# robertknight/ocrs-models

Hardware: AMD Instinct MI355X
Metric: detection train-step images/sec (higher is better)
Workload: dtype bf16

## Files before the change

include/ocrs_hip.h:

```cpp
#ifndef OCRS_HIP_H
#define OCRS_HIP_H

#ifdef __cplusplus
extern "C" {
#endif

#ifndef __HIP_PLATFORM_AMD__
typedef struct ihipStream_t* hipStream_t;
#endif

int ocrs_pack_frags(const float* src, int mode, int K, int M, int K2, long s1, long s2, long sm, void* out, int dtype, hipStream_t st);
long ocrs_pack_frags_bytes(int K, int M, int dtype);
int ocrs_pack_frags_multi(const long long* table, int n, long max_frag_threads, int dtype, hipStream_t st);

int ocrs_dwpw_fwd(const void* xa, const void* xb, int Ca, int Cb, const float* tra, const float* trb, const float* wdw, const void* wpk,
                  void* z, double* gstat, const float* gamma, void* pooled, int Cout, int N, int H, int W, int dtype, hipStream_t st);
long ocrs_dwpw_fwd_fin_supported(int Cin, int Cout, int dtype);
int ocrs_dwpw_fwd_fin(const void* xa, const void* xb, int Ca, int Cb, const float* tra, const float* trb, const float* wdw, const void* wpk, void* z,
                      double* gstat, unsigned* counter, long count, const float* bn_w, const float* bn_b, float eps, float momentum, float* tr, float* saved,
                      float* run_mean, float* run_var, long long* nbt, float lo, int Cout, int N, int H, int W, int dtype, hipStream_t st);
long ocrs_dwpw_fwd_pool_supported(int Cin, int Cout);
long ocrs_rs32_fwd_supported(int Ca, int Cb, int Cout, int dtype);
int ocrs_rs32_fwd(const float* xa, const float* xb, int Ca, int Cb, const float* tra, const float* trb, const float* wdw, const float* wpw, float* z,
                  double* gstat, const float* gamma, float* pooled, unsigned* counter, long count, const float* bn_w, const float* bn_b, float eps,
                  float momentum, float* tr, float* saved, float* run_mean, float* run_var, long long* nbt, float lo, int Cout, int N, int H, int W,
                  hipStream_t st);
long ocrs_rs32_bwd_supported(int Ca, int Cb, int Cout, int pooled, int dtype);
long ocrs_rs32_bwd_ws_floats(int Ca, int Cb, int Cout, int N, int H, int W);
int ocrs_rs32_bwd(const float* xa, const float* xb, int Ca, int Cb, const float* tra, const float* trb, const float* wdw, const float* wpw, const float* g1,
                  const float* g2, const float* z, const float* bn, const double* gsum, const float* gamma, const float* saved, float* dgamma, float* dbeta,
                  float* gxa, float* gxb, float* dwpw, float* dwdw, float* ws, const float* saved_a, double* gsum_a, const float* saved_b, double* gsum_b,
                  int pooled, int Cout, int N, int H, int W, hipStream_t st);
long ocrs_rs32_bwd_head_supported(int Ca, int Cb, int Cout, int dtype);
int ocrs_rs32_bwd_head(const float* xa, int Ca, const float* tra, const float* wdw, const float* wpw, const float* gl, const float* whead, const float* z,
                       const float* bn, const double* gsum, const float* gamma, const float* saved, float* dgamma, float* dbeta, float* gxa, float* dwpw,
                       float* dwdw, float* ws, const float* saved_a, double* gsum_a, int Cout, int N, int H, int W, hipStream_t st);
long ocrs_mm_fwd_supported(int Ca, int Cb, int Cout, int dtype);
long ocrs_mm_fwd_nparts(int Ca, int Cb, int Cout, int N, int H, int W);
int ocrs_mm_fwd(const void* xa, const void* xb, int Ca, int Cb, const float* tra, const float* trb, const float* wdw, const float* wpw, void* z,
                float* ws, const float* gamma, void* pooled, int Cout, int N, int H, int W, int dtype, hipStream_t st);
int ocrs_mm_fwd_fin(const void* xa, const void* xb, int Ca, int Cb, const float* tra, const float* trb, const float* wdw, const float* wpw, void* z, float* ws,
                    const float* gamma, void* pooled, unsigned* counter, long count, const float* bn_w, const float* bn_b, float eps, float momentum, float* tr,
                    float* saved, float* run_mean, float* run_var, long long* nbt, float lo, int Cout, int N, int H, int W, int dtype, hipStream_t st);
int ocrs_mm_fwd_fin_xu(const void* xu, const float* wexp, const float* tra, const float* wdw, const float* wpw, void* z, float* ws, unsigned* counter, long count,
                       const float* bn_w, const float* bn_b, float eps, float momentum, float* tr, float* saved, float* run_mean, float* run_var, long long* nbt,
                       float lo, int Cout, int N, int H, int W, int dtype, hipStream_t st);
int ocrs_bn_finalize_parts(const float* parts, int nparts, long count, int C, const float* gamma, const float* beta, float eps, float momentum,
                           float* tr, float* saved, float* run_mean, float* run_var, long long* nbt, float lo, hipStream_t st);
int ocrs_dwpw_c1_fwd(const float* img, const float* wdw, const float* wpw, void* z, double* gstat, int N, int H, int W, int dtype,
                     hipStream_t st);
long ocrs_dwpw_c1_u_supported(int N, int H, int W, int dtype);
int ocrs_dwpw_c1_fwd_u(const float* img, const float* wdw, const float* wpw, void* z, void* uplane, double* gstat, int N, int H, int W, int dtype,
                       hipStream_t st);
int ocrs_bn_finalize(const double* gstat, long count, int C, const float* gamma, const float* beta, float eps, float momentum, float* tr,
                     float* saved, float* run_mean, float* run_var, long long* nbt, float lo, hipStream_t st);
int ocrs_maxpool_fwd(const void* z, const float* tr, void* out, int C, int N, int H, int W, int raw, int dtype, hipStream_t st);
int ocrs_convt_fwd(const void* x, const float* tr, const void* wpk, const float* bias, void* out, int Cup, int Cout, int N, int h, int w,
                   int H, int W, int dtype, hipStream_t st);
long ocrs_rs32_convt_fwd_supported(int Cup, int Cout, int dtype);
int ocrs_rs32_convt_fwd(const float* x, const float* tr, const float* wt, const float* bias, float* out, int Cup, int Cout, int N, int h, int w, int H, int W,
                        hipStream_t st);
long ocrs_rs32_convt_dgrad_supported(int Cup, int Cout, int dtype);
int ocrs_rs32_convt_dgrad(const float* g, const float* wt, float* dx, const float* x, const float* tr, const float* saved, double* gsum, int Cup, int Cout, int N,
                          int h, int w, int H, int W, hipStream_t st);
int ocrs_head_fwd(const void* z, const float* tr, const float* w, const float* b, float* pred, long P, int dtype, hipStream_t st);

int ocrs_bn_bwd_reduce(const void* g1, const void* g2, int pooled, const void* z, const float* bn, const float* saved, double* gsum, int C,
                       int N, int H, int W, int dtype, hipStream_t st);
int ocrs_bn_bwd_finalize(const double* gsum, long count, int C, const float* gamma, const float* saved, float* coef, float* dgamma,
                         float* dbeta, hipStream_t st);
long ocrs_pw_bwd_ws_floats(int Cin, int Cout, int N, int H, int W);
int ocrs_pw_bwd(const void* xa, const void* xb, int Ca, int Cb, const float* tra, const float* trb, const float* wdw, const void* g1,
                const void* g2, int pooled, const void* z, const float* bn, const float* coef, const void* wpk_d, void* du, float* dwpw,
                float* ws, int Cout, int N, int H, int W, int dtype, hipStream_t st);
int ocrs_pw_bwd_fin(const void* xa, const void* xb, int Ca, int Cb, const float* tra, const float* trb, const float* wdw, const void* g1, const void* g2,
                    int pooled, const void* z, const float* bn, float* coef, const double* gsum, const float* gamma, const float* saved, float* dgamma,
                    float* dbeta, const void* wpk_d, void* du, float* dwpw, float* ws, int Cout, int N, int H, int W, int dtype, hipStream_t st);
long ocrs_pw_bwd_kernel(int Ca, int Cb, int Cout, int dtype);
long ocrs_dw_bwd_ws_floats(int C, int N, int H, int W);
int ocrs_dw_bwd(const void* xa, const void* xb, int Ca, int Cb, const float* tra, const float* trb, const float* wdw, const void* du,
                void* gxa, void* gxb, float* dwdw, float* ws, const float* saved_a, double* gsum_a, const float* saved_b, double* gsum_b,
                int N, int H, int W, int dtype, hipStream_t st);
long ocrs_mm_bwd_supported(int Ca, int Cb, int Cout, int dtype);
long ocrs_mm_bwd_ws_floats(int Ca, int Cb, int Cout, int N, int H, int W);
int ocrs_mm_bwd(const void* xa, const void* xb, int Ca, int Cb, const float* tra, const float* trb, const float* wdw, const float* wpw,
                const void* g1, const void* g2, int pooled, const void* z, const float* bn, const float* coef, void* gxa, void* gxb, float* dwpw,
                float* dwdw, float* ws, const float* saved_a, double* gsum_a, const float* saved_b, double* gsum_b, int Cout, int N, int H,
                int W, int dtype, hipStream_t st);
int ocrs_mm_bwd_fin(const void* xa, const void* xb, int Ca, int Cb, const float* tra, const float* trb, const float* wdw, const float* wpw, const void* g1,
                    const void* g2, int pooled, const void* z, const float* bn, const double* gsum, const float* gamma, const float* saved, float* dgamma,
                    float* dbeta, void* gxa, void* gxb, float* dwpw, float* dwdw, float* ws, const float* saved_a, double* gsum_a, const float* saved_b,
                    double* gsum_b, int Cout, int N, int H, int W, int dtype, hipStream_t st);
long ocrs_mm_bwd_head_supported(int Ca, int Cb, int Cout, int N, int H, int W, int dtype);
int ocrs_mm_bwd_fin_head(const void* xa, int Ca, const float* tra, const float* wdw, const float* wpw, const float* gl, const float* whead, const void* z,
                         const float* bn, const double* gsum, const float* gamma, const float* saved, float* dgamma, float* dbeta, void* gxa, float* dwpw,
                         float* dwdw, float* ws, const float* saved_a, double* gsum_a, int Cout, int N, int H, int W, int dtype, hipStream_t st);
int ocrs_mm_bwd_fin_xu(const void* xu, const float* wexp, const float* tra, const float* wdw, const float* wpw, const void* g1, const void* g2, const void* z,
                       const float* bn, const double* gsum, const float* gamma, const float* saved, float* dgamma, float* dbeta, void* gxa, float* dwpw,
                       float* dwdw, float* ws, const float* saved_a, double* gsum_a, int Cout, int N, int H, int W, int dtype, hipStream_t st);
int ocrs_dwpw_c1_bwd(const float* img, const float* wdw, const float* wpw, const void* g1, const void* g2, int pooled, const void* z,
                     const float* bn, const float* coef, double* acc64, int N, int H, int W, int dtype, hipStream_t st);
long ocrs_convt_bwd_ws_floats(int Cup, int Cout, int N, int h, int w, int dtype);
int ocrs_convt_bwd(const void* x, const float* tr, const void* g, const void* wpk_d, void* dx, float* dW, float* dbias, double* dbias64, float* ws,
                   const float* saved, double* gsum, int Cup, int Cout, int N, int h, int w, int H, int W, int dtype, hipStream_t st);
long ocrs_convt_bwd_stats_supported(int Cup, int Cout, int dtype);
long ocrs_convt_bwd_splittable(int Cup, int Cout, int dtype);
int ocrs_convt_bwd_parts(const void* x, const float* tr, const void* g, const void* wpk_d, void* dx, float* dW, float* dbias, double* dbias64, float* ws,
                         const float* saved, double* gsum, int Cup, int Cout, int N, int h, int w, int H, int W, int parts, int dtype, hipStream_t st);
int ocrs_dwpw_c1_fwd_us(const float* img, const float* wdw, const float* wpw, void* z, void* uplane, double* gstat, double* fsum, int N, int H, int W, int dtype,
                        hipStream_t st);
int ocrs_mm_bwd_fin_xu_c1(const void* xu, const float* wexp, const float* tra, const float* wdw, const float* wpw, const void* g1, const void* g2, const void* z,
                          const float* bn, const double* gsum, const float* gamma, const float* saved, float* dgamma, float* dbeta, float* dwpw, float* dwdw,
                          float* ws, const float* saved_a, double* gsum_a, const float* img, double* c1acc, int Cout, int N, int H, int W, int dtype,
                          hipStream_t st);
int ocrs_c1_bwd_fin(const double* c1acc, const double* fsum, const float* coef, const float* wexp, double* acc64, hipStream_t st);
int ocrs_bwd_defer_begin(double* scratch, long ndoubles);
int ocrs_bwd_defer_flush(hipStream_t st);
int ocrs_head_bwd(const void* z, const float* tr, const float* w, const float* pred, const float* gpred, void* gy, double* acc64,
                  const float* saved, double* gsum, long P, int dtype, hipStream_t st);
int ocrs_head_bwd_gl(const void* z, const float* tr, const float* w, const float* pred, const float* gpred, float* gl, double* acc64,
                     const float* saved, double* gsum, long P, int dtype, hipStream_t st);
int ocrs_head_bwd_loss(const void* z, const float* tr, const float* w, const float* pred, const float* target, const float* lpx, const unsigned char* cls,
                       const void* state, const float* gout, float* gl, double* acc64, const float* saved, double* gsum, long P, int dtype,
                       hipStream_t st);

long ocrs_loss_state_bytes(void);
long ocrs_loss_hist_bytes(void);
int ocrs_balanced_bce_fwd(const float* pred, const float* target, float* lpx, unsigned char* cls, void* state, void* hist, float* loss_out,
                          long P, hipStream_t st);
int ocrs_balanced_bce_bwd(const float* pred, const float* target, const float* lpx, const unsigned char* cls, const void* state,
                          const float* gout, float* gpred, long P, hipStream_t st);
int ocrs_fold64_multi(const int* table, int nrows, float* dst, const double* src, hipStream_t st);

int ocrs_conv_igemm(const void* x, int ldx, const void* wpk, void* out, int ldo, const float* bias, int relu, double* gstat, int Cin, int M, int N,
                    int Hi, int Wi, int Ho, int Wo, int KH, int KW, int padh, int padw, int dtype, hipStream_t st);
long ocrs_conv_igemm_kernel(int ldx, int ldo, int Cin, int M, int Hi, int Wi, int Ho, int Wo, int KH, int KW, int padh, int padw, int dtype);
long ocrs_wgrad_gemm_x3_ws_floats(int CA, int CB, long P);
int ocrs_wgrad_gemm_x3(const float* A, int ldA, int CA, const float* B, int ldB, int CB, float* dW, float* ws, long P, hipStream_t st);
int ocrs_gemm_x3(const float* X, int ldx, int K, const float* Wm, int ldw, int km, const float* bias, float* out, int ldo, int M, long P, int Kw,
                 hipStream_t st);
long ocrs_gemm_x3p_supported(int ldx, int K, int ldo, int M, long P);
int ocrs_gemm_x3p(const float* X, int ldx, int K, const void* wpk, const float* bias, float* out, int ldo, int M, long P, hipStream_t st);
int ocrs_gemm_x3p_tiles(const float* X, int ldx, int K, const void* wpk, const float* bias, float* out, int ldo, int M, long P, int ntw, hipStream_t st);
long ocrs_wgrad_gather_ws_floats(int CA, int CB, int ntaps, long P, int dtype);
int ocrs_wgrad_gather(const void* A, int ldA, int CA, const float* trA, const void* B, int ldB, int CB, float* dW, float* ws, int N, int hA,
                      int wA, int HB, int WB, int stride, int padh, int padw, int KH, int KW, int dtype, hipStream_t st);
long ocrs_conv3x3_wgrad_ws_floats(int Cout, int Cin, int N, int H, int W);
int ocrs_conv3x3_wgrad(const void* dz, int Cout, const void* x, int Cin, float* dW, float* ws, int N, int H, int W, int dtype, hipStream_t st);
int ocrs_conv0_fwd(const float* img, const float* w, const float* bias, void* out, int N, int H, int W, int dtype, hipStream_t st);
int ocrs_conv0_bwd(const float* img, const float* w, const float* bias, const void* g, float* dW, float* db, int N, int H, int W, int dtype,
                   hipStream_t st);
int ocrs_act_pool_fwd(const void* z, const float* tr, void* out, int C, int N, int H, int W, int PH, int PW, int dtype, hipStream_t st);
int ocrs_rec_bn_reduce(const void* g, const void* z, const float* bn, const float* saved, double* gsum, int C, int N, int H, int W, int PH, int PW,
                       int dtype, hipStream_t st);
int ocrs_dz_apply(const void* g, const void* z, const float* bn, const float* coef, void* dz, int C, int N, int H, int W, int PH, int PW, int dtype,
                  float* dsum , hipStream_t st);
int ocrs_avgpool_fwd(const void* z, const float* tr, float* seq, int C, int N, int H, int W, int dtype, hipStream_t st);
int ocrs_avgpool_bn_reduce(const float* gseq, const void* z, const float* saved, double* gsum, int C, int N, int H, int W, int dtype, hipStream_t st);
int ocrs_avgpool_dz(const float* gseq, const void* z, const float* coef, void* dz, int C, int N, int H, int W, int dtype, hipStream_t st);
int ocrs_col_sum(const void* a, int ld, int C, float* out, long rows, int dtype, hipStream_t st);
int ocrs_gru_layer_fwd(const float* gi, const float* whh_pk, const float* bhh, float* out, float* saved, int T, int N, hipStream_t st);
int ocrs_gru_layer_bwd(const float* dout, const float* saved, const float* out, const float* whhT_pk, float* dgi, float* dgh, float* dhz, int T,
                       int N, hipStream_t st);
long ocrs_gru_seq_supported(int N);
long ocrs_gru_seq_sync_words(int N);
long ocrs_gru_seq_ws_floats(int N);
int ocrs_gru_seq_fwd(const float* gi, const float* whh, const float* bhh, float* out, float* saved, int T, int N, unsigned* sync, unsigned* err, float* xws,
                     int exact, hipStream_t st);
int ocrs_gru_seq_bwd(const float* dout, const float* saved, const float* out, const float* whh, float* dgi, float* dgh, int T, int N, unsigned* sync,
                     unsigned* err, float* xws, int exact, float* dbih, float* dbhh, hipStream_t st);
int ocrs_gru_seq_status(const unsigned* err, hipStream_t st);
int ocrs_log_softmax_fwd(const void* logits, float* out, long rows, int C, int ld, int dtype, hipStream_t st);
int ocrs_log_softmax_bwd(const float* lp, const float* g, void* dlogits, long rows, int C, int ld, int dtype, hipStream_t st);
int ocrs_ctc_fwd(const float* lp, const int* targets, const long long* in_len, const long long* tg_len, float* alpha, float* nll, float* loss,
                 int T, int N, int C, int Lpad, int Smax, hipStream_t st);
int ocrs_ctc_bwd(const float* lp, const int* targets, const long long* in_len, const long long* tg_len, const float* alpha, const float* nll,
                 const float* gout, float* grad, int T, int N, int C, int Lpad, int Smax, hipStream_t st);
int ocrs_ctc_fwd_ab(const float* lp, const int* targets, const long long* in_len, const long long* tg_len, float* alpha, float* beta, float* nll,
                    float* loss, int T, int N, int C, int Lpad, int Smax, hipStream_t st);
int ocrs_ctc_grad_ab(const float* lp, const int* targets, const long long* in_len, const long long* tg_len, const float* alpha, const float* beta,
                     const float* nll, const float* gout, float* grad, int T, int N, int C, int Lpad, int Smax, hipStream_t st);
int ocrs_ctc_fwd_h16(const float* lp, const int* targets, const long long* in_len, const long long* tg_len, void* alpha16, float* rowmax, float* nll,
                     float* loss, int T, int N, int C, int Lpad, int Smax, hipStream_t st);
int ocrs_ctc_bwd_h16(const float* lp, const int* targets, const long long* in_len, const long long* tg_len, const void* alpha16, const float* rowmax,
                     const float* nll, const float* gout, float* grad, int T, int N, int C, int Lpad, int Smax, hipStream_t st);
int ocrs_ctc_greedy_decode(const float* lp, const long long* in_len, int* amax, int* labels, int* lens, int T, int N, int C, hipStream_t st);
long ocrs_edit_distance_ws_bytes(int N, int pa);
int ocrs_edit_distance(const int* a, const long long* a_len, int pa, const int* b, const long long* b_len, int pb, const int* codes, int ncodes,
                       void* ws, int* dist, int N, hipStream_t st);
long ocrs_ctc_cer_ws_bytes(int T, int N, int Lpitch);
int ocrs_ctc_cer_update(const float* lp, const long long* in_len, const int* targets, const long long* tgt_len, const int* codes, void* ws,
                        long long* state, int* dist, int T, int N, int C, int Lpitch, hipStream_t st);

int ocrs_transform_image_u8(const void* img_u8, void* out, long n, int dtype, hipStream_t st);
int ocrs_collate_pad(const void* packed, const long long* offs, const int* widths, void* out, int B, int H, int Wpad, int kind, int dtype,
                     hipStream_t st);
int ocrs_resize_aa(const float* in, float* ws, float* out, int planes, int h, int w, int oh, int ow, hipStream_t st);
long ocrs_resize_aa_ws_floats(int planes, int h, int ow);

long ocrs_augment_det_ws_floats(int B);
int ocrs_augment_det(const void* img_u8, const void* mask, const long long* offs, const int* params, float* ws, void* img_out, float* mask_out,
                     int B, int max_h, int max_w, int OH, int OW, int mask_kind, int dtype, hipStream_t st);
long ocrs_augment_lines_ws_floats(int B, long inter_floats, long hpass_floats);
int ocrs_augment_lines(const void* crops, const void* masks, const long long* offs, const int* params, float* ws, long inter_floats, void* out, int B,
                       int max_ih, int max_iw, int OH, int Wpad, int kind, int clamp, int dtype, hipStream_t st);

long ocrs_cc_quads_capacity(int H, int W);
long ocrs_cc_quads_ws_bytes(int B, int H, int W);
int ocrs_cc_quads(const void* mask, int kind, float threshold, int B, int H, int W, int* ncomp, float* quads, int* labels, void* ws,
                  hipStream_t st);
long ocrs_box_match_ws_bytes(int B, long cap_t, int nbkt);
int ocrs_box_match_metrics(const float* pred_quads, const int* n_pred, long cap_p, const float* target_quads, const int* n_target, long cap_t, int B,
                           int nbkt, double* out, void* ws, hipStream_t st);
long ocrs_mask_metrics_ws_bytes(int B, int H, int W);
int ocrs_mask_metrics(const void* pred, int pred_kind, const void* target, int target_kind, float threshold, int B, int H, int W, double* out, void* ws,
                      hipStream_t st);

int ocrs_binarize_resize_nearest(const float* prob, unsigned char* out, int B, int h, int w, int H, int W, float threshold, hipStream_t st);
int ocrs_expand_quads(const float* quads, float* out, const int* counts, int B, long cap, float dist, hipStream_t st);
int ocrs_crop_plan(const float* quads, const int* count, long cap, int output_height, int* plan, long long* totals, hipStream_t st);
int ocrs_rectify_crops(const unsigned char* page, int H, int W, const float* quads, const int* plan, const long long* totals, long max_tiles, float* packed,
                       long packed_floats, hipStream_t st);
long ocrs_resize_aa_packed_ws_floats(long hpass_floats);
int ocrs_resize_aa_packed(const float* packed, const int* plan, const int* count, long cap, const long long* chunks, int nchunks, int max_batch, float* ws,
                          long ws_floats, float* out, long out_floats, int output_height, hipStream_t st);

long ocrs_text_lines_ws_bytes(long cap);
int ocrs_line_links(const float* quads, const int* count, long cap, float max_gap, float min_cos, int* next_word, void* ws, long ws_bytes, hipStream_t st);
int ocrs_line_rank(const int* count, long cap, const int* next_word, void* ws, long ws_bytes, hipStream_t st);
int ocrs_line_order(const int* count, long cap, int* n_lines, int* line_of_word, int* word_order, int* line_offsets, void* ws, long ws_bytes, hipStream_t st);
int ocrs_line_quads(const float* quads, const int* count, long cap, const int* n_lines, const int* line_offsets, const int* word_order, float* line_quads,
                    void* ws, long ws_bytes, hipStream_t st);

int ocrs_binarize_resize_pages(const float* prob, const int* page_sizes, unsigned char* out, int B, int h, int w, int Hmax, int Wmax, float threshold,
                               hipStream_t st);
int ocrs_gather_page_quads(const float* quads, const int* counts, int B, long cap, float* out, int* page_of_word, int* word_offs, long out_cap, hipStream_t st);
long ocrs_text_lines_pages_ws_bytes(long cap, int B);
int ocrs_line_links_pages(const float* quads, const int* word_offs, int B, long cap, float max_gap, float min_cos, int* next_word, void* ws, long ws_bytes,
                          hipStream_t st);
int ocrs_line_rank_pages(const int* word_offs, int B, long cap, const int* next_word, void* ws, long ws_bytes, hipStream_t st);
int ocrs_line_order_pages(const int* word_offs, int B, long cap, int* n_lines, int* line_of_word, int* word_order, int* line_offsets, int* line_page_offs,
                          int* page_of_line, void* ws, long ws_bytes, hipStream_t st);
int ocrs_line_quads_pages(const float* quads, const int* word_offs, int B, long cap, const int* n_lines, const int* line_offsets, const int* word_order,
                          float* line_quads, void* ws, long ws_bytes, hipStream_t st);
int ocrs_rectify_crops_pages(const unsigned char* pages, long pages_bytes, const long long* page_offs, const int* page_sizes, int B, const float* quads,
                             const int* page_of_quad, const int* plan, const long long* totals, long max_tiles, float* packed, long packed_floats,
                             hipStream_t st);

long ocrs_tile_batch_ws_floats(int T, int max_th, int ow);
int ocrs_tile_batch(const unsigned char* pages, long pages_bytes, const long long* page_offs, const int* page_sizes, int B, const int* tiles, int T, int max_th,
                    float* ws, long ws_floats, float* out, int oh, int ow, hipStream_t st);
#define OCRS_TILES_AXIS_MAX 64
int ocrs_binarize_resize_tiles(const float* prob, int T, int h, int w, const int* tiles, const int* tile_offs, const int* page_sizes, const int* grids,
                               const int* row_cuts, const int* col_cuts, int max_axis, unsigned char* out, int B, int Hmax, int Wmax, float threshold,
                               hipStream_t st);

long ocrs_reading_order_ws_bytes(long cap, int B);
int ocrs_reading_relation(const float* line_quads, const int* n_lines, const int* line_page_offs , int B, long cap, unsigned* before,
                          void* ws, long ws_bytes, hipStream_t st);
int ocrs_reading_peel(const int* n_lines, const int* line_page_offs, int B, long cap, const unsigned* before, int* line_order, void* ws, long ws_bytes,
                      hipStream_t st);
int ocrs_reading_blocks(const int* n_lines, const int* line_page_offs, int B, long cap, float block_gap, const int* line_order, int* new_block, void* ws,
                        long ws_bytes, hipStream_t st);

int ocrs_ctc_decode_spans(const float* lp, const long long* in_len, int* amax, float* amax_lp, int T, int N, int C, long row0, int ld, int* labels, int* t0, int* t1,
                          float* peak, int* lens, hipStream_t st);
int ocrs_char_boxes(const float* quads, const int* plan, long cap, long rows, int ld, const int* lens, const int* t0, const int* t1, float* s0, float* s1,
                    float* char_quads, hipStream_t st);
int ocrs_word_chars(const float* words, long wcap, const float* line_quads, const int* n_lines, long cap, const int* line_offsets, const int* word_order,
                    const int* plan, long rows, int ld, const int* labels, const int* lens, const float* s0, const float* s1, int space, int* word_chars,
                    hipStream_t st);

int ocrs_line_spines(const float* words, long wcap, const int* n_lines, long cap, const int* line_offsets, const int* word_order, float* spine, float* line_dims,
                     hipStream_t st);
int ocrs_crop_plan_dims(const float* line_dims, const int* count, long cap, int output_height, int* plan, long long* totals, hipStream_t st);
int ocrs_rectify_chain(const unsigned char* page, int H, int W, const float* spine, const float* line_dims, const int* line_offsets, long wcap, const int* plan,
                       const long long* totals, long max_tiles, float* packed, long packed_floats, hipStream_t st);
int ocrs_rectify_chain_pages(const unsigned char* pages, long pages_bytes, const long long* page_offs, const int* page_sizes, int B, const float* spine,
                             const float* line_dims, const int* line_offsets, long wcap, const int* page_of_line, const int* plan, const long long* totals,
                             long max_tiles, float* packed, long packed_floats, hipStream_t st);
int ocrs_char_boxes_chain(const float* spine, const float* line_dims, const int* line_offsets, long wcap, const int* plan, long cap, long rows, int ld,
                          const int* lens, const int* t0, const int* t1, float* s0, float* s1, float* char_quads, hipStream_t st);
int ocrs_word_chars_chain(const float* spine, long wcap, const int* n_lines, long cap, const int* line_offsets, const int* word_order, const int* plan, long rows,
                          int ld, const int* labels, const int* lens, const float* s0, const float* s1, int space, int* word_chars, hipStream_t st);

int ocrs_turn_page_u8(const unsigned char* src, int H, int W, int k, unsigned char* dst, hipStream_t st);
int ocrs_turn_quads(const float* quads, long n, const int* count, int H, int W, int k, int inverse, float* out, hipStream_t st);
int ocrs_orient_votes(const float* quads, long n, const int* count, float min_aspect, int sample, double* votes, int* picks, hipStream_t st);
int ocrs_path_confidence(const float* log_probs, int T, int B, int C, const int* steps, double* scores, hipStream_t st);

long ocrs_ctc_beam_ws_bytes(int T, int N, int W);
long ocrs_ctc_align_ws_bytes(int T, int N, int Lmax);
int ocrs_ctc_beam_decode(const float* lp, const long long* in_len, int T, int N, int C, int W, long row0, int ld, int* labels, int* lens, float* score, void* ws,
                         long ws_bytes, hipStream_t st);
int ocrs_ctc_beam_decode_lm(const float* lp, const long long* in_len, int T, int N, int C, int W, const float* gain, int order, long row0, int ld, int* labels,
                            int* lens, float* score, float* lm_score, void* ws, long ws_bytes, hipStream_t st);
int ocrs_ctc_align_spans(const float* lp, const long long* in_len, int T, int N, int C, long row0, int ld, const int* labels, int* lens, int* t0, int* t1,
                         float* peak, void* ws, long ws_bytes, hipStream_t st);

int ocrs_eval_pair_iou(const float* pred_quads, const int* pred_offs, const float* gt_quads, const int* gt_offs, const unsigned char* gt_ignore,
                       const long long* pair_offs, int B, long P, long G, long n_pairs, long max_pairs, double* iou, int* ign_hit, hipStream_t st);
long ocrs_eval_match_ws_bytes(long P, long G);
int ocrs_eval_match(const double* iou, const long long* pair_offs, const int* pred_offs, const int* gt_offs, const unsigned char* gt_ignore,
                    const int* ign_hit, int B, long P, long G, long n_pairs, double min_iou, int* gt_of_pred, int* pred_of_gt, double* iou_of_pred, void* ws,
                    hipStream_t st);
int ocrs_eval_text_update(const int* pred_offs, const int* gt_offs, const unsigned char* gt_ignore, int B, long P, long G, int max_page_preds,
                          const int* gt_of_pred, const int* pred_of_gt, const int* pred_text, const int* pred_text_offs, long n_pred_text,
                          const int* gt_text, const int* gt_text_offs, long n_gt_text, int* bnd, int* dist, int* flags, long long* state, hipStream_t st);

int ocrs_layout_dropout_mask(unsigned char* mask, long n, float p, long seed, int site, hipStream_t st);
int ocrs_layout_embed(const float* boxes, const float* rates, float* out, long rows, hipStream_t st);
long ocrs_layout_attn_supported(int S);
int ocrs_layout_attn_fwd(const float* qkv, float* out, int S, int W, float p, long seed, int site, hipStream_t st);
int ocrs_layout_attn_bwd(const float* qkv, const float* dout, float* dqkv, int S, int W, float p, long seed, int site, hipStream_t st);
int ocrs_layout_ln_fwd(const float* x, const float* a, const float* gamma, const float* beta, float* y, float* stat, long rows, float eps, float p, long seed,
                       int site, hipStream_t st);
long ocrs_layout_ln_bwd_ws_floats(long rows);
int ocrs_layout_ln_bwd(const float* dy1, const float* dy2, const float* x, const float* a, const float* stat, const float* gamma, float* ds, float* da,
                       float* dgamma, float* dbeta, float* ws, long rows, float p, long seed, int site, hipStream_t st);
int ocrs_layout_relu_drop_fwd(float* h, long n, int relu, float p, long seed, int site, hipStream_t st);
int ocrs_layout_relu_drop_bwd(const float* g, const float* h, float* out, long n, float p, hipStream_t st);
long ocrs_layout_col_sum_ws_floats(int C, long rows);
int ocrs_layout_col_sum(const float* a, int ld, int C, int Cout, float* out, float* ws, long rows, hipStream_t st);
int ocrs_layout_head_out(const float* logits, int ld, float* out, long rows, int probs, hipStream_t st);
int ocrs_layout_head_grad_in(const float* g, float* dlog, int ld, long rows, hipStream_t st);
long ocrs_layout_loss_ws_bytes(void);
int ocrs_layout_loss(const float* pred, const float* target, float pos_weight, int pred_is_prob, float* loss, float* dlogits, long long* counts, void* ws,
                     long rows, hipStream_t st);
int ocrs_layout_stats_update(const long long* counts, double* sums, hipStream_t st);
int ocrs_weblayout_batch(const double* coords, const int* para, const long long* page_off, const double* viewport, int P, const int* pages,
                         const double* jitter, int N, int W, int normalize, float* boxes, float* labels, hipStream_t st);
int ocrs_line_mask(const int* vertices, const long long* vertex_offs, const int* vertex_counts, const int* sizes, const long long* out_offs,
                   void* out_u8, int n, int max_h, hipStream_t st);
int ocrs_line_batch(const void* pixels_u8, const long long* pixel_offs, const int* sizes, const int* vertices, const long long* vertex_offs,
                    const int* vertex_counts, int N, const int* indices, int B, int max_h, const long long* batch_offs, void* out_crops_u8,
                    void* out_masks_u8, hipStream_t st);

int ocrs_shrink_polygons(const int* vertices, const long long* vertex_offs, const int* vertex_counts, int n, double dist, int* ws, double* out_xy,
                         int* out_vertices, int* out_counts, int* out_rows, hipStream_t st);
int ocrs_page_batch(const void* pixels_u8, const long long* pixel_offs, const int* sizes, const int* vertices, long n_vertices, const int* polys,
                    int n_polys, const long long* band_offs, const int* bands, int N, const int* indices, int B, int max_h, int max_w,
                    const long long* batch_offs, void* out_pages_u8, void* out_masks_u8, hipStream_t st);

int ocrs_opt_chunk(void);
int ocrs_clip_grad_norm(const long long* table, const int* chunks, int nchunks, float max_norm, double* sumsq, float* norm_out,
                        float* coef_out, int scale_in_place, hipStream_t st);
int ocrs_adam_step(const long long* table, const int* chunks, int nchunks, float b1, float b2, float eps, float step_size, float bc2_sqrt,
                   const float* gscale, hipStream_t st);
int ocrs_adam_step_dev(const long long* table, const int* chunks, int nchunks, double b1, double b2, float eps, double lr, float* step,
                       const float* gscale, hipStream_t st);
int ocrs_fill_f32(float* p, float v, long n, hipStream_t st);

int ocrs_prof_enable(int on);
long ocrs_prof_count(void);
int ocrs_prof_read(float* ms, long first, long n, hipStream_t st);
int ocrs_cu_hog(int blocks, int micros, hipStream_t st);

#ifdef __cplusplus
}
#endif
#endif
```

ocrs_models_amd/csrc/det_common.h:

```cpp
#pragma once
#include "common.h"

struct PixIdx {
    int n, h, w;
};
__device__ __forceinline__ PixIdx decode_pixel(long p, int H, int W) {
    PixIdx r;
    const unsigned q = (unsigned)p, uw = (unsigned)W, uh = (unsigned)H;
    const unsigned row = q / uw;
    r.w = (int)(q - row * uw);
    r.n = (int)(row / uh);
    r.h = (int)(row - (unsigned)r.n * uh);
    return r;
}

struct PixIter {
    int n, h, w, sn, sh, sw, H, W;
    __device__ __forceinline__ PixIter(long first, long stride, int H_, int W_) : H(H_), W(W_) {
        const PixIdx a = decode_pixel(first, H_, W_), s = decode_pixel(stride, H_, W_);
        n = a.n; h = a.h; w = a.w;
        sn = s.n; sh = s.h; sw = s.w;
    }
    __device__ __forceinline__ PixIdx cur() const {
        PixIdx r;
        r.n = n; r.h = h; r.w = w;
        return r;
    }
    __device__ __forceinline__ void next() {
        w += sw;
        if (w >= W) { w -= W; ++h; }
        h += sh;
        if (h >= H) { h -= H; ++n; }
        n += sn;
    }
};

struct Tiling {
    int H, W, tw_shift, tiles_x, tiles_y, ntiles;
};
static inline Tiling make_tiling(int N, int H, int W, int TP) {
    Tiling t;
    int sh = 0;
    while ((1 << sh) < W && (1 << sh) < 32 && (1 << sh) < TP) ++sh;
    t.H = H; t.W = W; t.tw_shift = sh;
    const int TW = 1 << sh, TH = TP >> sh;
    t.tiles_x = (W + TW - 1) / TW;
    t.tiles_y = (H + TH - 1) / TH;
    t.ntiles = N * t.tiles_x * t.tiles_y;
    return t;
}
struct TileOrg {
    int n, h0, w0;
};
__device__ __forceinline__ TileOrg tile_origin(const Tiling& tg, int TP, int tile) {
    TileOrg o;
    const int tpi = tg.tiles_x * tg.tiles_y;
    o.n = tile / tpi;
    const int r = tile - o.n * tpi;
    const int ty = r / tg.tiles_x;
    o.h0 = ty * (TP >> tg.tw_shift);
    o.w0 = (r - ty * tg.tiles_x) << tg.tw_shift;
    return o;
}
__device__ __forceinline__ bool tile_pixel(const Tiling& tg, const TileOrg& o, int pxl, PixIdx& px) {
    px.n = o.n;
    px.h = o.h0 + (pxl >> tg.tw_shift);
    px.w = o.w0 + (pxl & ((1 << tg.tw_shift) - 1));
    return px.h < tg.H && px.w < tg.W;
}
__device__ __forceinline__ long pix_linear(const PixIdx& px, int H, int W) { return ((long)px.n * H + px.h) * W + px.w; }

template <int TW, int TH>
struct HaloTile {
    static constexpr int HW_ = TW + 2, HH_ = TH + 2, HP = HW_ * HH_;
};
struct Tiling2 {
    int H, W, tiles_x, tiles_y, ntiles;
};
static inline Tiling2 make_tiling2(int N, int H, int W, int TW, int TH) {
    Tiling2 t;
    t.H = H; t.W = W;
    t.tiles_x = (W + TW - 1) / TW;
    t.tiles_y = (H + TH - 1) / TH;
    t.ntiles = N * t.tiles_x * t.tiles_y;
    return t;
}
template <int TW, int TH>
__device__ __forceinline__ TileOrg tile_origin2(const Tiling2& tg, int tile) {
    TileOrg o;
    const int tpi = tg.tiles_x * tg.tiles_y;
    o.n = tile / tpi;
    const int r = tile - o.n * tpi;
    const int ty = r / tg.tiles_x;
    o.h0 = ty * TH;
    o.w0 = (r - ty * tg.tiles_x) * TW;
    return o;
}

struct Nb9 {
    float v[9];
    unsigned ok;
};
__device__ __forceinline__ void nb9_issue(Nb9& nb, const float* __restrict__ img, const PixIdx& px, int H, int W, bool active) {
    const long rowc = ((long)px.n * H + px.h) * W + px.w;
    nb.ok = 0;
#pragma unroll
    for (int k = 0; k < 9; ++k) {
        const int dy = k / 3 - 1, dx = k % 3 - 1;
        const bool ok = active && (unsigned)(px.h + dy) < (unsigned)H && (unsigned)(px.w + dx) < (unsigned)W;
        nb.v[k] = img[ok ? rowc + (long)dy * W + dx : 0];
        nb.ok |= ok ? 1u << k : 0u;
    }
}
__device__ __forceinline__ void nb9_finish(const Nb9& nb, float (&v)[9]) {
#pragma unroll
    for (int k = 0; k < 9; ++k) v[k] = (nb.ok >> k & 1u) ? nb.v[k] : 0.f;
}

template <int TW, int TH>
struct TileIter {
    int n, ty, tx, sn, sy, sx, tiles_x, tiles_y;
    __device__ __forceinline__ TileIter(const Tiling2& tg, long first, long step) {
        const int tpi = tg.tiles_x * tg.tiles_y;
        tiles_x = tg.tiles_x;
        tiles_y = tg.tiles_y;
        n = (int)first / tpi;
        const int r = (int)first - n * tpi;
        ty = r / tiles_x;
        tx = r - ty * tiles_x;
        sn = (int)step / tpi;
        const int rs = (int)step - sn * tpi;
        sy = rs / tiles_x;
        sx = rs - sy * tiles_x;
    }
    __device__ __forceinline__ TileOrg org() const {
        TileOrg o;
        o.n = n;
        o.h0 = ty * TH;
        o.w0 = tx * TW;
        return o;
    }
    __device__ __forceinline__ void next() {
        tx += sx;
        if (tx >= tiles_x) {
            tx -= tiles_x;
            ++ty;
        }
        ty += sy;
        if (ty >= tiles_y) {
            ty -= tiles_y;
            ++n;
        }
        n += sn;
    }
};

template <class T>
struct Src2 {
    const T* a;
    const T* b;
    int Ca, Cb;
};

template <class T>
__device__ __forceinline__ const T* src_ptr(const Src2<T>& s, long pix, int c0) {
    return (c0 < s.Ca) ? s.a + pix * s.Ca + c0 : s.b + pix * s.Cb + (c0 - s.Ca);
}

__device__ __forceinline__ void apply_tr8(float (&v)[8], const float* tr, int C, int c0) {
#pragma unroll
    for (int i = 0; i < 8; ++i) v[i] = fmaxf(fmaf(v[i], tr[c0 + i], tr[C + c0 + i]), tr[2 * C + c0 + i]);
}

template <int CG>
__device__ __forceinline__ int xs_swz(int item) {
    return item ^ (((item >> 4) & 1) * CG);
}

template <class T>
__device__ __forceinline__ void fill_tr8(float* s_tr8, const Src2<T>& x, const float* __restrict__ tra, const float* __restrict__ trb, int CIN,
                                         int tid) {
    for (int i = tid; i < 3 * CIN; i += 256) {
        const int g = i / 24, r = (i - g * 24) >> 3, c = g * 8 + (i & 7);
        s_tr8[i] = c < x.Ca ? tra[r * x.Ca + c] : trb[r * x.Cb + (c - x.Ca)];
    }
}
__device__ __forceinline__ float max_lo(float v, float lo) {
    float r;
    asm("v_max_f32 %0, %1, %2" : "=v"(r) : "v"(v), "v"(lo));
    return r;
}

template <class T, int CG, int TW, int TH, int NT = 256 >
struct HaloStager {
    using HT = HaloTile<TW, TH>;
    static constexpr int NITEMS = HT::HP * CG;
    static constexpr int PLANE = NITEMS * 4;
    static constexpr int NIT = (NITEMS + NT - 1) / NT;
    __device__ static __forceinline__ void put(float* xs, int it, const float (&v)[8]) {
        const int o = xs_swz<CG>(it) * 4;
        store4(xs + o, v[0], v[1], v[2], v[3]);
        store4(xs + PLANE + o, v[4], v[5], v[6], v[7]);
    }
    int hyx[NIT];
    int poff[NIT];
    int cg;
    __device__ __forceinline__ HaloStager(int tid, int W) {
        cg = tid % CG;
#pragma unroll
        for (int j = 0; j < NIT; ++j) {
            const int hp = (tid + j * NT) / CG;
            const int hy = hp / HT::HW_, hx = hp - hy * HT::HW_;
            hyx[j] = hy | (hx << 16);
            poff[j] = hy * W + hx;
        }
    }
    __device__ __forceinline__ void stage(const Src2<T>& x, const float* s_tr8, int ch0, const TileOrg& org, int H, int W, float* xs,
                                          int tid) const {
        const int c0 = ch0 + cg * 8;
        const bool from_a = c0 < x.Ca;
        const long corner = ((long)org.n * H + (org.h0 - 1)) * W + (org.w0 - 1);
        const long offa = corner * x.Ca, offb = corner * x.Cb;
        const T* base = (from_a ? x.a + c0 : x.b + (c0 - x.Ca)) + (from_a ? offa : offb);
        const int pitch = from_a ? x.Ca : x.Cb;
        const float* tp = s_tr8 + (c0 >> 3) * 24;
        float sc[8], sh[8], lo[8];
        load8(tp, sc);
        load8(tp + 8, sh);
        load8(tp + 16, lo);
        const float zero8[8] = {0.f, 0.f, 0.f, 0.f, 0.f, 0.f, 0.f, 0.f};
#pragma unroll
        for (int j = 0; j < NIT; ++j) {
            if (NITEMS % NT != 0 && j == NIT - 1 && tid + j * NT >= NITEMS) break;
            const int h = org.h0 - 1 + (hyx[j] & 0xffff), w = org.w0 - 1 + (hyx[j] >> 16);
            if ((unsigned)h < (unsigned)H && (unsigned)w < (unsigned)W) {
                float v[8];
                load8(base + __umul24(poff[j], pitch), v);
#pragma unroll
                for (int i = 0; i < 8; ++i) v[i] = max_lo(fmaf(v[i], sc[i], sh[i]), lo[i]);
                put(xs, tid + j * NT, v);
            } else
                put(xs, tid + j * NT, zero8);
        }
    }

    struct Pending {
        Raw8<T> raw[NIT];
        unsigned ok;
    };
    __device__ __forceinline__ void issue(Pending& pd, const Src2<T>& x, int ch0, const TileOrg& org, int H, int W, int tid) const {
        const int c0 = ch0 + cg * 8;
        const bool from_a = c0 < x.Ca;
        const long corner = ((long)org.n * H + (org.h0 - 1)) * W + (org.w0 - 1);
        const long offa = corner * x.Ca, offb = corner * x.Cb;
        const T* base = (from_a ? x.a + c0 : x.b + (c0 - x.Ca)) + (from_a ? offa : offb);
        const int pitch = from_a ? x.Ca : x.Cb;
        pd.ok = 0;
        const T* dummy = from_a ? x.a : x.b;
#pragma unroll
        for (int j = 0; j < NIT; ++j) {
            const int h = org.h0 - 1 + (hyx[j] & 0xffff), w = org.w0 - 1 + (hyx[j] >> 16);
            const bool ok = (unsigned)h < (unsigned)H && (unsigned)w < (unsigned)W && (NITEMS % NT == 0 || j < NIT - 1 || tid + j * NT < NITEMS);
            pd.raw[j] = load8_raw(ok ? base + __umul24(poff[j], pitch) : dummy);
            pd.ok |= ok ? 1u << j : 0u;
        }
    }
    __device__ __forceinline__ void commit(const Pending& pd, const float* s_tr8, int ch0, float* xs, int tid) const {
        const float* tp = s_tr8 + ((ch0 >> 3) + cg) * 24;
        float sc[8], sh[8], lo[8];
        load8(tp, sc);
        load8(tp + 8, sh);
        load8(tp + 16, lo);
        const float zero8[8] = {0.f, 0.f, 0.f, 0.f, 0.f, 0.f, 0.f, 0.f};
#pragma unroll
        for (int j = 0; j < NIT; ++j) {
            if (NITEMS % NT != 0 && j == NIT - 1 && tid + j * NT >= NITEMS) break;
            if (pd.ok & (1u << j)) {
                float v[8];
                unpack8(pd.raw[j], v);
#pragma unroll
                for (int i = 0; i < 8; ++i) v[i] = max_lo(fmaf(v[i], sc[i], sh[i]), lo[i]);
                put(xs, tid + j * NT, v);
            } else
                put(xs, tid + j * NT, zero8);
        }
    }
};

template <int CG, int TW, int TH, bool SWZ = true>
__device__ __forceinline__ void dw_from_lds(const float* xs, const float* s_w , int CIN, int c0, int cg, int ty, int tx,
                                            float (&u)[8]) {
    constexpr int HWp = TW + 2;
    constexpr int PLANE = HaloTile<TW, TH>::HP * CG * 4;
    const int item0 = (ty * HWp + tx) * CG + cg;
#pragma unroll
    for (int i = 0; i < 8; ++i) u[i] = 0.f;
#pragma unroll
    for (int t = 0; t < 9; ++t) {
        float v[8], wv[8];
        const int it = item0 + ((t / 3) * HWp + (t % 3)) * CG;
        const float* q = xs + (SWZ ? xs_swz<CG>(it) : it) * 4;
        const float4 lo4 = *reinterpret_cast<const float4*>(q), hi4 = *reinterpret_cast<const float4*>(q + PLANE);
        v[0] = lo4.x; v[1] = lo4.y; v[2] = lo4.z; v[3] = lo4.w;
        v[4] = hi4.x; v[5] = hi4.y; v[6] = hi4.z; v[7] = hi4.w;
        load8(s_w + t * CIN + c0, wv);
#pragma unroll
        for (int i = 0; i < 8; ++i) u[i] = fmaf(wv[i], v[i], u[i]);
    }
}

template <int CG, int TW, int TH>
__device__ __forceinline__ void dw2_from_lds(const float* xs, const float* s_w , int CIN, int c0, int cg, int ty, int tx,
                                             float (&u0)[8], float (&u1)[8]) {
    constexpr int HWp = TW + 2;
    constexpr int PLANE = HaloTile<TW, TH>::HP * CG * 4;
    const int item0 = (ty * HWp + tx) * CG + cg;
#pragma unroll
    for (int i = 0; i < 8; ++i) u0[i] = u1[i] = 0.f;
#pragma unroll
    for (int r = 0; r < 3; ++r) {
        float w[3][8];
#pragma unroll
        for (int c = 0; c < 3; ++c) load8(s_w + (r * 3 + c) * CIN + c0, w[c]);
#pragma unroll
        for (int c = 0; c < 4; ++c) {
            const float* q = xs + xs_swz<CG>(item0 + (r * HWp + c) * CG) * 4;
            const float4 lo4 = *reinterpret_cast<const float4*>(q), hi4 = *reinterpret_cast<const float4*>(q + PLANE);
            const float v[8] = {lo4.x, lo4.y, lo4.z, lo4.w, hi4.x, hi4.y, hi4.z, hi4.w};
#pragma unroll
            for (int i = 0; i < 8; ++i) {
                if (c < 3) u0[i] = fmaf(w[c][i], v[i], u0[i]);
                if (c > 0) u1[i] = fmaf(w[c - 1][i], v[i], u1[i]);
            }
        }
    }
}

template <class T>
struct GradSrc {
    const T* g1;
    const T* g2;
    int pooled;
};

template <class T>
__device__ __forceinline__ void load_ghat8(const GradSrc<T>& gs, const T* z, int C, const float* bn, long p, const PixIdx& px, int H,
                                           int W, int c0, float (&gh)[8], float (&zv)[8]) {
    load8(z + p * C + c0, zv);
    float y[8];
#pragma unroll
    for (int i = 0; i < 8; ++i) y[i] = fmaf(zv[i], bn[c0 + i], bn[C + c0 + i]);
    if (!gs.pooled) {
        float g[8];
        load8(gs.g1 + p * C + c0, g);
        if (gs.g2) {
            float g2[8];
            load8(gs.g2 + p * C + c0, g2);
#pragma unroll
            for (int i = 0; i < 8; ++i) g[i] += g2[i];
        }
#pragma unroll
        for (int i = 0; i < 8; ++i) gh[i] = y[i] > 0.f ? g[i] : 0.f;
        return;
    }
    const int Hp = H >> 1, Wp = W >> 1;
#pragma unroll
    for (int i = 0; i < 8; ++i) gh[i] = 0.f;
    if (px.h >= 2 * Hp || px.w >= 2 * Wp) return;
    const int ph = px.h >> 1, pw = px.w >> 1;
    const long pp = ((long)px.n * Hp + ph) * Wp + pw;
    float g[8];
    load8(gs.g1 + pp * C + c0, g);
    if (gs.g2) {
        float g2[8];
        load8(gs.g2 + pp * C + c0, g2);
#pragma unroll
        for (int i = 0; i < 8; ++i) g[i] += g2[i];
    }
    const int own = ((px.h & 1) << 1) | (px.w & 1);
    bool win[8];
#pragma unroll
    for (int i = 0; i < 8; ++i) win[i] = y[i] > 0.f;
    const long base = ((long)px.n * H + 2 * ph) * W + 2 * pw;
#pragma unroll
    for (int k = 0; k < 4; ++k) {
        if (k == own) continue;
        float zo[8];
        load8(z + (base + (long)(k >> 1) * W + (k & 1)) * C + c0, zo);
#pragma unroll
        for (int i = 0; i < 8; ++i) {
            const float yo = fmaxf(fmaf(zo[i], bn[c0 + i], bn[C + c0 + i]), 0.f);
            const float ym = fmaxf(y[i], 0.f);
            win[i] = win[i] && (k < own ? ym > yo : ym >= yo);
        }
    }
#pragma unroll
    for (int i = 0; i < 8; ++i) gh[i] = win[i] ? g[i] : 0.f;
}

template <class T>
struct GhatPend {
    Raw8<T> z, g1, g2, zo0, zo1, zo2;
};
template <class T>
__device__ __forceinline__ void issue_ghat8(GhatPend<T>& pd, const GradSrc<T>& gs, const T* z, int C, long p, const PixIdx& px, int H, int W,
                                            int c0, bool act) {
    const bool pooled = gs.pooled != 0;
    const int Hp = H >> 1, Wp = W >> 1;
    const int ph = px.h >> 1, pw = px.w >> 1;
    const bool inw = act && (!pooled || (px.h < 2 * Hp && px.w < 2 * Wp));
    const long pg = pooled ? ((long)px.n * Hp + ph) * Wp + pw : p;
    const T* g2b = gs.g2 ? gs.g2 : gs.g1;
    pd.z = load8_raw(act ? z + p * C + c0 : z);
    pd.g1 = load8_raw(inw ? gs.g1 + pg * C + c0 : gs.g1);
    pd.g2 = load8_raw(inw ? g2b + pg * C + c0 : g2b);
    const bool wz = inw && pooled;
    const int own = ((px.h & 1) << 1) | (px.w & 1);
    const long base = ((long)px.n * H + 2 * ph) * W + 2 * pw;
    const int k0 = own <= 0 ? 1 : 0, k1 = own <= 1 ? 2 : 1, k2 = own <= 2 ? 3 : 2;
    pd.zo0 = load8_raw(wz ? z + (base + (long)(k0 >> 1) * W + (k0 & 1)) * C + c0 : z);
    pd.zo1 = load8_raw(wz ? z + (base + (long)(k1 >> 1) * W + (k1 & 1)) * C + c0 : z);
    pd.zo2 = load8_raw(wz ? z + (base + (long)(k2 >> 1) * W + (k2 & 1)) * C + c0 : z);
}
template <class T>
__device__ __forceinline__ void finish_ghat8(const GhatPend<T>& pd, const GradSrc<T>& gs, int C, const float* bn, const PixIdx& px, int H, int W,
                                             int c0, float (&gh)[8], float (&zv)[8]) {
    unpack8(pd.z, zv);
    float y[8], g[8];
#pragma unroll
    for (int i = 0; i < 8; ++i) y[i] = fmaf(zv[i], bn[c0 + i], bn[C + c0 + i]);
    unpack8(pd.g1, g);
    if (gs.g2) {
        float g2[8];
        unpack8(pd.g2, g2);
#pragma unroll
        for (int i = 0; i < 8; ++i) g[i] += g2[i];
    }
    if (!gs.pooled) {
#pragma unroll
        for (int i = 0; i < 8; ++i) gh[i] = y[i] > 0.f ? g[i] : 0.f;
        return;
    }
    const int Hp = H >> 1, Wp = W >> 1;
    const bool inw = px.h < 2 * Hp && px.w < 2 * Wp;
    const int own = ((px.h & 1) << 1) | (px.w & 1);
    bool win[8];
#pragma unroll
    for (int i = 0; i < 8; ++i) win[i] = inw && y[i] > 0.f;
#pragma unroll
    for (int j = 0; j < 3; ++j) {
        float zo[8];
        unpack8(j == 0 ? pd.zo0 : (j == 1 ? pd.zo1 : pd.zo2), zo);
#pragma unroll
        for (int i = 0; i < 8; ++i) {
            const float yo = fmaxf(fmaf(zo[i], bn[c0 + i], bn[C + c0 + i]), 0.f);
            const float ym = fmaxf(y[i], 0.f);
            win[i] = win[i] && (j < own ? ym > yo : ym >= yo);
        }
    }
#pragma unroll
    for (int i = 0; i < 8; ++i) gh[i] = win[i] ? g[i] : 0.f;
}

struct BnFin {
    const double* gsum;
    const float* gamma;
    const float* saved;
    float* dgamma;
    float* dbeta;
    long count;
};
__device__ __forceinline__ void bn_fin_coef(const BnFin& fin, int COUT, float* s_cf , int tid, int nt, bool writer) {
    for (int c = tid; c < COUT; c += nt) {
        const double s1 = fin.gsum[c], s2 = fin.gsum[COUT + c];
        const double m1 = s1 / (double)fin.count, m2 = s2 / (double)fin.count;
        const double mean = fin.saved[c], rstd = fin.saved[COUT + c];
        const double A = (double)fin.gamma[c] * rstd;
        s_cf[c] = (float)A;
        s_cf[COUT + c] = (float)(-A * rstd * m2);
        s_cf[2 * COUT + c] = (float)(A * (-m1 + mean * rstd * m2));
        if (writer) {
            fin.dgamma[c] = (float)s2;
            fin.dbeta[c] = (float)s1;
        }
    }
}

struct BwdLast {
    double* raw;
    unsigned* counter;
    double *gsum_a, *gsum_b;
    const float *saved_a, *saved_b;
    int Ca;
    int mode;
};
constexpr int BWD_LAST_SLOTS = 8;
__device__ __forceinline__ void bwd_last_add(const BwdLast& bl, int CIN, int c, int which, float v) {
    atomicAdd(bl.raw + ((blockIdx.x + blockIdx.y) & (BWD_LAST_SLOTS - 1)) * 2 * CIN + which * CIN + c, (double)v);
}
__device__ __forceinline__ void bwd_last_finish(const BwdLast& bl, int CIN, const float* __restrict__ tra, const float* __restrict__ trb, int tid, int nt,
                                                int* s_flag) {
    asm volatile("s_waitcnt vmcnt(0)" ::: "memory");
    __syncthreads();
    if (tid == 0) *s_flag = __hip_atomic_fetch_add(bl.counter, 1u, __ATOMIC_RELAXED, __HIP_MEMORY_SCOPE_AGENT) == gridDim.x * gridDim.y - 1 ? 1 : 0;
    __syncthreads();
    if (*s_flag == 0) return;
    for (int c = tid; c < CIN; c += nt) {
        double S1 = 0.0, S2 = 0.0;
        for (int k = 0; k < BWD_LAST_SLOTS; ++k) {
            double* r = bl.raw + k * 2 * CIN;
            S1 += __hip_atomic_load(r + c, __ATOMIC_RELAXED, __HIP_MEMORY_SCOPE_AGENT);
            S2 += __hip_atomic_load(r + CIN + c, __ATOMIC_RELAXED, __HIP_MEMORY_SCOPE_AGENT);
            __hip_atomic_store(r + c, 0.0, __ATOMIC_RELAXED, __HIP_MEMORY_SCOPE_AGENT);
            __hip_atomic_store(r + CIN + c, 0.0, __ATOMIC_RELAXED, __HIP_MEMORY_SCOPE_AGENT);
        }
        const bool in_a = c < bl.Ca;
        double* gs = in_a ? bl.gsum_a : bl.gsum_b;
        if (!gs) continue;
        const int cc = in_a ? c : c - bl.Ca, Cs = in_a ? bl.Ca : CIN - bl.Ca;
        const float* sv = in_a ? bl.saved_a : bl.saved_b;
        const double mean = sv[cc], rstd = sv[Cs + cc];
        gs[cc] += S1;
        if (bl.mode == 0) {
            const float* tr = in_a ? tra : trb;
            const double sc = tr[cc], sh = tr[Cs + cc];
            if (sc != 0.0) gs[Cs + cc] += rstd * ((S2 - sh * S1) / sc - mean * S1);
        } else {
            gs[Cs + cc] += (double)((float)S2 * sv[Cs + cc]);
        }
    }
    if (tid == 0) __hip_atomic_store(bl.counter, 0u, __ATOMIC_RELAXED, __HIP_MEMORY_SCOPE_AGENT);
}

struct FwdFin {
    unsigned* counter;
    long count;
    const float *gamma, *beta;
    float eps, momentum;
    float *tr, *saved, *run_mean, *run_var;
    long long* nbt;
    float lo;
};
__device__ __forceinline__ void bn_finalize_channel(double sum, double sumsq, long count, int c, int C, const float* gamma, const float* beta, float eps, float momentum,
                                                    float* tr, float* saved, float* run_mean, float* run_var, float lo) {
    const double mean = sum / (double)count;
    double var = sumsq / (double)count - mean * mean;
    if (var < 0) var = 0;
    const float rstd = (float)(1.0 / sqrt(var + (double)eps));
    const float sc = gamma[c] * rstd;
    tr[c] = sc;
    tr[C + c] = beta[c] - (float)mean * sc;
    tr[2 * C + c] = lo;
    saved[c] = (float)mean;
    saved[C + c] = rstd;
    if (run_mean) {
        const double unb = count > 1 ? var * (double)count / (double)(count - 1) : var;
        run_mean[c] = (1.f - momentum) * run_mean[c] + momentum * (float)mean;
        run_var[c] = (1.f - momentum) * run_var[c] + momentum * (float)unb;
    }
}

__device__ __forceinline__ void bn_finalize_last_block(const FwdFin& fin, const double* gstat, int C, int tid, int nt, int* s_flag) {
    if (!fin.counter) return;
    asm volatile("s_waitcnt vmcnt(0)" ::: "memory");
    __syncthreads();
    if (tid == 0) *s_flag = __hip_atomic_fetch_add(fin.counter, 1u, __ATOMIC_RELAXED, __HIP_MEMORY_SCOPE_AGENT) == gridDim.x - 1 ? 1 : 0;
    __syncthreads();
    if (*s_flag == 0) return;
    for (int c = tid; c < C; c += nt) {
        const double sum = __hip_atomic_load(gstat + c, __ATOMIC_RELAXED, __HIP_MEMORY_SCOPE_AGENT);
        const double sq = __hip_atomic_load(gstat + C + c, __ATOMIC_RELAXED, __HIP_MEMORY_SCOPE_AGENT);
        bn_finalize_channel(sum, sq, fin.count, c, C, fin.gamma, fin.beta, fin.eps, fin.momentum, fin.tr, fin.saved, fin.run_mean, fin.run_var, fin.lo);
    }
    if (tid == 0) {
        if (fin.nbt) *fin.nbt += 1;
        __hip_atomic_store(fin.counter, 0u, __ATOMIC_RELAXED, __HIP_MEMORY_SCOPE_AGENT);
    }
}
```

ocrs_models_amd/csrc/det_head.hip:

```cpp
#include "det_common.h"
#include "loss_state.h"

template <class T>
__global__ __launch_bounds__(256) void k_head_fwd(const T* __restrict__ z, const float* __restrict__ tr, const float* __restrict__ w,
                                                  const float* __restrict__ b, float* __restrict__ pred, long P) {
    float wv[8], sc[8], sh[8], lo[8];
#pragma unroll
    for (int i = 0; i < 8; ++i) {
        wv[i] = w[i];
        sc[i] = tr[i];
        sh[i] = tr[8 + i];
        lo[i] = tr[16 + i];
    }
    const float bias = b[0];
    for (long p = (long)blockIdx.x * 256 + threadIdx.x; p < P; p += (long)gridDim.x * 256) {
        float v[8];
        load8(z + p * 8, v);
        float s = bias;
#pragma unroll
        for (int i = 0; i < 8; ++i) s = fmaf(wv[i], fmaxf(fmaf(v[i], sc[i], sh[i]), lo[i]), s);
        pred[p] = 1.f / (1.f + __expf(-s));
    }
}

template <class T>
__global__ __launch_bounds__(256) void k_head_bwd(const T* __restrict__ z, const float* __restrict__ tr, const float* __restrict__ w,
                                                  const float* __restrict__ pred, const float* __restrict__ gpred, T* __restrict__ gy,
                                                  double* __restrict__ acc64 , const float* __restrict__ saved ,
                                                  double* __restrict__ gsum , long P, float* __restrict__ gl_out ) {
    __shared__ float s_slots[4 * 25];
    float wv[8], sc[8], sh[8], lo[8], mu[8], acc[9] = {0, 0, 0, 0, 0, 0, 0, 0, 0}, st1[8], st2[8];
#pragma unroll
    for (int i = 0; i < 8; ++i) {
        wv[i] = w[i];
        sc[i] = tr[i];
        sh[i] = tr[8 + i];
        lo[i] = tr[16 + i];
        mu[i] = gsum ? saved[i] : 0.f;
        st1[i] = st2[i] = 0.f;
    }
    for (long p = (long)blockIdx.x * 256 + threadIdx.x; p < P; p += (long)gridDim.x * 256) {
        const float pr = pred[p];
        const float gl = gpred[p] * (1.f - pr) * pr;
        float v[8], o[8];
        load8(z + p * 8, v);
#pragma unroll
        for (int i = 0; i < 8; ++i) {
            const float pre = fmaf(v[i], sc[i], sh[i]);
            const float xv = fmaxf(pre, lo[i]);
            acc[i] = fmaf(gl, xv, acc[i]);
            o[i] = gl * wv[i];
            const float gh = pre > 0.f ? Elem<T>::round(o[i]) : 0.f;
            st1[i] += gh;
            st2[i] = fmaf(gh, v[i] - mu[i], st2[i]);
        }
        acc[8] += gl;
        if (gl_out) gl_out[p] = gl;
        else store8(gy + p * 8, o);
    }
    float all[25];
#pragma unroll
    for (int i = 0; i < 9; ++i) all[i] = acc[i];
#pragma unroll
    for (int i = 0; i < 8; ++i) {
        all[9 + i] = st1[i];
        all[17 + i] = st2[i];
    }
    const float tot = block_sum_det<25>(all, s_slots);
    if (threadIdx.x < 9) atomicAdd(&acc64[threadIdx.x], (double)tot);
    if (gsum && threadIdx.x >= 9 && threadIdx.x < 25) {
        const int i = threadIdx.x - 9;
        atomicAdd(&gsum[i], (double)(i < 8 ? tot : tot * saved[8 + (i - 8)]));
    }
}

template <class T>
__global__ __launch_bounds__(256) void k_head_bwd_loss(const T* __restrict__ z, const float* __restrict__ tr, const float* __restrict__ w,
                                                       const float* __restrict__ pred, const float* __restrict__ target,
                                                       const float* __restrict__ lpx, const unsigned char* __restrict__ cls,
                                                       const LossState* __restrict__ stt, const float* __restrict__ gout,
                                                       double* __restrict__ acc64 , const float* __restrict__ saved ,
                                                       double* __restrict__ gsum , long P, float* __restrict__ gl_out ) {
    __shared__ float s_slots[4 * 25];
    float wv[8], sc[8], sh[8], lo[8], mu[8], acc[9] = {0, 0, 0, 0, 0, 0, 0, 0, 0}, st1[8], st2[8];
#pragma unroll
    for (int i = 0; i < 8; ++i) {
        wv[i] = w[i];
        sc[i] = tr[i];
        sh[i] = tr[8 + i];
        lo[i] = tr[16 + i];
        mu[i] = saved[i];
        st1[i] = st2[i] = 0.f;
    }
    const unsigned t0 = stt->prefix[0], t1 = stt->prefix[1];
    const float f0 = stt->frac[0], f1 = stt->frac[1];
    const float s = gout[0] * stt->inv2k;
    const long nq = P >> 2;
    for (long q = (long)blockIdx.x * 256 + threadIdx.x; q < nq; q += (long)gridDim.x * 256) {
        const float4 p4 = reinterpret_cast<const float4*>(pred)[q], t4 = reinterpret_cast<const float4*>(target)[q];
        const float4 l4 = reinterpret_cast<const float4*>(lpx)[q];
        const unsigned c4 = reinterpret_cast<const unsigned*>(cls)[q];
        float v[4][8];
#pragma unroll
        for (int e = 0; e < 4; ++e) load8(z + (q * 4 + e) * 8, v[e]);
        const float pe[4] = {p4.x, p4.y, p4.z, p4.w}, te[4] = {t4.x, t4.y, t4.z, t4.w}, le[4] = {l4.x, l4.y, l4.z, l4.w};
        float gle[4];
#pragma unroll
        for (int e = 0; e < 4; ++e) {
            const unsigned c = (c4 >> (8 * e)) & 0xffu;
            const float pr = pe[e];
            float gp = 0.f;
            if (c) {
                const unsigned key = loss_key(le[e]);
                const unsigned thr = c == 1 ? t0 : t1;
                const float wgt = key > thr ? 1.f : (key == thr ? (c == 1 ? f0 : f1) : 0.f);
                if (wgt != 0.f) {
                    const float t = fminf(fmaxf(te[e], 0.f), 1.f);
                    gp = s * wgt * (pr - t) / fmaxf((1.f - pr) * pr, 1e-12f);
                }
            }
            const float gl = gp * (1.f - pr) * pr;
            gle[e] = gl;
#pragma unroll
            for (int i = 0; i < 8; ++i) {
                const float pre = fmaf(v[e][i], sc[i], sh[i]);
                const float xv = fmaxf(pre, lo[i]);
                acc[i] = fmaf(gl, xv, acc[i]);
                const float gh = pre > 0.f ? Elem<T>::round(gl * wv[i]) : 0.f;
                st1[i] += gh;
                st2[i] = fmaf(gh, v[e][i] - mu[i], st2[i]);
            }
            acc[8] += gl;
        }
        reinterpret_cast<float4*>(gl_out)[q] = make_float4(gle[0], gle[1], gle[2], gle[3]);
    }
    float all[25];
#pragma unroll
    for (int i = 0; i < 9; ++i) all[i] = acc[i];
#pragma unroll
    for (int i = 0; i < 8; ++i) {
        all[9 + i] = st1[i];
        all[17 + i] = st2[i];
    }
    const float tot = block_sum_det<25>(all, s_slots);
    if (threadIdx.x < 9) atomicAdd(&acc64[threadIdx.x], (double)tot);
    if (threadIdx.x >= 9 && threadIdx.x < 25) {
        const int i = threadIdx.x - 9;
        atomicAdd(&gsum[i], (double)(i < 8 ? tot : tot * saved[8 + (i - 8)]));
    }
}

static int head_bwd_impl(const void* z, const float* tr, const float* w, const float* pred, const float* gpred, void* gy, float* gl, double* acc64,
                         const float* saved, double* gsum, long P, int dtype, hipStream_t st) {
    OCRS_CHECK_ARG(z && tr && w && pred && gpred && (gy || gl) && acc64 && P > 0 && (!gsum || saved));
    int grid = ew_grid(P);
    if (grid > 1024) grid = 1024;
    if (dtype == 1)
        hipLaunchKernelGGL(k_head_bwd<bf16>, dim3(grid), dim3(256), 0, st, (const bf16*)z, tr, w, pred, gpred, (bf16*)gy, acc64, saved, gsum, P, gl);
    else
        hipLaunchKernelGGL(k_head_bwd<float>, dim3(grid), dim3(256), 0, st, (const float*)z, tr, w, pred, gpred, (float*)gy, acc64, saved, gsum, P, gl);
    OCRS_LAUNCH_CHECK();
    return OCRS_OK;
}

extern "C" {

int ocrs_head_fwd(const void* z, const float* tr, const float* w, const float* b, float* pred, long P, int dtype, hipStream_t st) {
    OCRS_CHECK_ARG(z && tr && w && b && pred && P > 0);
    const int grid = ew_grid(P);
    if (dtype == 1)
        hipLaunchKernelGGL(k_head_fwd<bf16>, dim3(grid), dim3(256), 0, st, (const bf16*)z, tr, w, b, pred, P);
    else
        hipLaunchKernelGGL(k_head_fwd<float>, dim3(grid), dim3(256), 0, st, (const float*)z, tr, w, b, pred, P);
    OCRS_LAUNCH_CHECK();
    return OCRS_OK;
}

int ocrs_head_bwd(const void* z, const float* tr, const float* w, const float* pred, const float* gpred, void* gy, double* acc64,
                  const float* saved, double* gsum, long P, int dtype, hipStream_t st) {
    OCRS_CHECK_ARG(gy);
    return head_bwd_impl(z, tr, w, pred, gpred, gy, nullptr, acc64, saved, gsum, P, dtype, st);
}
int ocrs_head_bwd_gl(const void* z, const float* tr, const float* w, const float* pred, const float* gpred, float* gl, double* acc64,
                     const float* saved, double* gsum, long P, int dtype, hipStream_t st) {
    OCRS_CHECK_ARG(gl);
    return head_bwd_impl(z, tr, w, pred, gpred, nullptr, gl, acc64, saved, gsum, P, dtype, st);
}
int ocrs_head_bwd_loss(const void* z, const float* tr, const float* w, const float* pred, const float* target, const float* lpx, const unsigned char* cls,
                       const void* state, const float* gout, float* gl, double* acc64, const float* saved, double* gsum, long P, int dtype,
                       hipStream_t st) {
    OCRS_CHECK_ARG(z && tr && w && pred && target && lpx && cls && state && gout && gl && acc64 && saved && gsum && P > 0 && P % 4 == 0);
    int grid = ew_grid(P / 4);
    if (dtype == 1)
        hipLaunchKernelGGL(k_head_bwd_loss<bf16>, dim3(grid), dim3(256), 0, st, (const bf16*)z, tr, w, pred, target, lpx, cls, (const LossState*)state,
                           gout, acc64, saved, gsum, P, gl);
    else
        hipLaunchKernelGGL(k_head_bwd_loss<float>, dim3(grid), dim3(256), 0, st, (const float*)z, tr, w, pred, target, lpx, cls,
                           (const LossState*)state, gout, acc64, saved, gsum, P, gl);
    OCRS_LAUNCH_CHECK();
    return OCRS_OK;
}

}
```

ocrs_models_amd/csrc/loss_optim.hip:

```cpp
#include "common.h"

#include "loss_state.h"

constexpr int LOSS_MAXB = 1024;
constexpr int LOSS_HIST_WORDS = 2 * 2048;
struct LossParts {
    unsigned long long cnt[LOSS_MAXB][2];
    double sum[LOSS_MAXB][2];
};
__device__ __forceinline__ LossParts* loss_parts(unsigned* hist) { return reinterpret_cast<LossParts*>(hist + LOSS_HIST_WORDS); }

__device__ __forceinline__ float log1p_neg(float p) {
    const float u = 1.f - p;
    if (u <= 0.f) return -__builtin_inff();
    return logf(u) - ((u - 1.f) + p) / u;
}

template <int VEC>
struct Quad {
    float v[VEC];
};
template <int VEC>
__device__ __forceinline__ Quad<VEC> ldq(const float* p, long q) {
    Quad<VEC> r;
    if constexpr (VEC == 4) {
        const float4 a = reinterpret_cast<const float4*>(p)[q];
        r.v[0] = a.x; r.v[1] = a.y; r.v[2] = a.z; r.v[3] = a.w;
    } else
        r.v[0] = p[q];
    return r;
}
template <int VEC>
__device__ __forceinline__ void stq(float* p, long q, const Quad<VEC>& r) {
    if constexpr (VEC == 4)
        reinterpret_cast<float4*>(p)[q] = make_float4(r.v[0], r.v[1], r.v[2], r.v[3]);
    else
        p[q] = r.v[0];
}
template <int VEC>
struct QuadB {
    unsigned char v[VEC];
};
template <int VEC>
__device__ __forceinline__ QuadB<VEC> ldqb(const unsigned char* p, long q) {
    QuadB<VEC> r;
    if constexpr (VEC == 4) {
        const unsigned a = reinterpret_cast<const unsigned*>(p)[q];
        r.v[0] = a & 255; r.v[1] = (a >> 8) & 255; r.v[2] = (a >> 16) & 255; r.v[3] = a >> 24;
    } else
        r.v[0] = p[q];
    return r;
}
template <int VEC>
__device__ __forceinline__ void stqb(unsigned char* p, long q, const QuadB<VEC>& r) {
    if constexpr (VEC == 4)
        reinterpret_cast<unsigned*>(p)[q] = r.v[0] | (r.v[1] << 8) | (r.v[2] << 16) | ((unsigned)r.v[3] << 24);
    else
        p[q] = r.v[0];
}

template <int VEC>
__global__ __launch_bounds__(256) void k_bce_fwd(const float* __restrict__ pred, const float* __restrict__ target, float* __restrict__ lpx,
                                                 unsigned char* __restrict__ cls, unsigned* __restrict__ hist, long P) {
    __shared__ unsigned s_h[LOSS_HIST_WORDS];
    for (int i = threadIdx.x; i < LOSS_HIST_WORDS; i += 256) s_h[i] = 0;
    __syncthreads();
    unsigned long long np = 0, nn = 0;
    const long nq = P / VEC;
    for (long q = (long)blockIdx.x * 256 + threadIdx.x; q < nq; q += (long)gridDim.x * 256) {
        const Quad<VEC> pq = ldq<VEC>(pred, q), tq = ldq<VEC>(target, q);
        Quad<VEC> lq;
        QuadB<VEC> cq;
#pragma unroll
        for (int e = 0; e < VEC; ++e) {
            const float p = pq.v[e], t0 = tq.v[e];
            const unsigned char c = t0 > 0.5f ? 1 : (t0 < 0.5f ? 2 : 0);
            const float t = fminf(fmaxf(t0, 0.f), 1.f);
            lq.v[e] = -(t * fmaxf(logf(p), -100.f) + (1.f - t) * fmaxf(log1p_neg(p), -100.f));
            cq.v[e] = c;
            np += c == 1;
            nn += c == 2;
        }
        stq<VEC>(lpx, q, lq);
        stqb<VEC>(cls, q, cq);
#pragma unroll
        for (int e = 0; e < VEC; ++e)
            if (cq.v[e]) atomicAdd(&s_h[(cq.v[e] - 1) * 2048 + (loss_key(lq.v[e]) >> 20)], 1u);
    }
    if (VEC > 1 && blockIdx.x == 0 && threadIdx.x < P - nq * VEC) {
        const long i = nq * VEC + threadIdx.x;
        const float p = pred[i], t0 = target[i];
        const unsigned char c = t0 > 0.5f ? 1 : (t0 < 0.5f ? 2 : 0);
        const float t = fminf(fmaxf(t0, 0.f), 1.f);
        const float l = -(t * fmaxf(logf(p), -100.f) + (1.f - t) * fmaxf(log1p_neg(p), -100.f));
        lpx[i] = l;
        cls[i] = c;
        np += c == 1;
        nn += c == 2;
        if (c) atomicAdd(&s_h[(c - 1) * 2048 + (loss_key(l) >> 20)], 1u);
    }
    __shared__ unsigned s_cnt[2];
    if (threadIdx.x < 2) s_cnt[threadIdx.x] = 0;
    __syncthreads();
    for (int o = 32; o > 0; o >>= 1) {
        np += __shfl_xor(np, o, 64);
        nn += __shfl_xor(nn, o, 64);
    }
    if ((threadIdx.x & 63) == 0) {
        atomicAdd(&s_cnt[0], (unsigned)np);
        atomicAdd(&s_cnt[1], (unsigned)nn);
    }
    __syncthreads();
    if (threadIdx.x < 2) loss_parts(hist)->cnt[blockIdx.x][threadIdx.x] = s_cnt[threadIdx.x];
    for (int i = threadIdx.x; i < LOSS_HIST_WORDS; i += 256)
        if (s_h[i]) atomicAdd(&hist[i], s_h[i]);
}

__device__ __forceinline__ void pass_bits(int pass, int& shift, int& nb) {
    shift = pass == 0 ? 20 : (pass == 1 ? 10 : 0);
    nb = pass == 0 ? 2048 : 1024;
}

template <int VEC>
__global__ __launch_bounds__(256) void k_select_hist(const float* __restrict__ lpx, const unsigned char* __restrict__ cls,
                                                     const LossState* __restrict__ stt, unsigned* __restrict__ hist , int pass,
                                                     long P) {
    __shared__ unsigned s_h[2 * 2048];
    for (int i = threadIdx.x; i < 4096; i += 256) s_h[i] = 0;
    __syncthreads();
    int shift, nb;
    pass_bits(pass, shift, nb);
    const unsigned pf0 = stt->prefix[0], pf1 = stt->prefix[1];
    const int hs = shift + (pass == 0 ? 11 : 10);
    double s0 = 0.0, s1 = 0.0;
    auto visit = [&](unsigned char c, float v) {
        if (!c) return;
        const unsigned key = loss_key(v);
        const unsigned pf = c == 1 ? pf0 : pf1;
        const unsigned up = key >> hs;
        if (pass == 0 || up == pf) atomicAdd(&s_h[(c - 1) * 2048 + ((key >> shift) & (nb - 1))], 1u);
        if (pass == 2 && up > pf) {
            if (c == 1) s0 += (double)v;
            else s1 += (double)v;
        }
    };
    const long nq = P / VEC;
    const long stride = (long)gridDim.x * 256;
    long q = (long)blockIdx.x * 256 + threadIdx.x;
    for (; q + 3 * stride < nq; q += 4 * stride) {
        QuadB<VEC> cq[4];
        Quad<VEC> lq[4];
#pragma unroll
        for (int u = 0; u < 4; ++u) {
            cq[u] = ldqb<VEC>(cls, q + u * stride);
            lq[u] = ldq<VEC>(lpx, q + u * stride);
        }
#pragma unroll
        for (int u = 0; u < 4; ++u)
#pragma unroll
            for (int e = 0; e < VEC; ++e) visit(cq[u].v[e], lq[u].v[e]);
    }
    for (; q < nq; q += stride) {
        const QuadB<VEC> cq = ldqb<VEC>(cls, q);
        const Quad<VEC> lq = ldq<VEC>(lpx, q);
#pragma unroll
        for (int e = 0; e < VEC; ++e) visit(cq.v[e], lq.v[e]);
    }
    if (VEC > 1 && blockIdx.x == 0 && threadIdx.x < P - nq * VEC) visit(cls[nq * VEC + threadIdx.x], lpx[nq * VEC + threadIdx.x]);
    __syncthreads();
    for (int i = threadIdx.x; i < 4096; i += 256)
        if (s_h[i]) atomicAdd(&hist[i], s_h[i]);
    if (pass == 2) {
        __shared__ double s_sum[2][4];
        for (int o = 32; o > 0; o >>= 1) {
            s0 += __shfl_xor(s0, o, 64);
            s1 += __shfl_xor(s1, o, 64);
        }
        if ((threadIdx.x & 63) == 0) {
            s_sum[0][threadIdx.x >> 6] = s0;
            s_sum[1][threadIdx.x >> 6] = s1;
        }
        __syncthreads();
        if (threadIdx.x < 2) loss_parts(hist)->sum[blockIdx.x][threadIdx.x] = (s_sum[threadIdx.x][0] + s_sum[threadIdx.x][1]) + (s_sum[threadIdx.x][2] + s_sum[threadIdx.x][3]);
    }
}

__global__ __launch_bounds__(256) void k_select_scan(LossState* __restrict__ stt, unsigned* __restrict__ hist, int pass, int nblk, float* __restrict__ loss_out) {
    __shared__ unsigned long long s_sum[256];
    __shared__ double s_d[256];
    __shared__ unsigned long long s_need[2], s_ties[2], s_k;
    __shared__ int s_bin[2];
    int shift, nb;
    pass_bits(pass, shift, nb);
    const int per = nb / 256;
    const int tid = threadIdx.x;
    LossParts* lp = loss_parts(hist);
    auto block_sum_u64 = [&](unsigned long long v) -> unsigned long long {
        __syncthreads();
        s_sum[tid] = v;
        __syncthreads();
        for (int o = 128; o > 0; o >>= 1) {
            if (tid < o) s_sum[tid] += s_sum[tid + o];
            __syncthreads();
        }
        return s_sum[0];
    };
    auto block_sum_f64 = [&](double v) -> double {
        __syncthreads();
        s_d[tid] = v;
        __syncthreads();
        for (int o = 128; o > 0; o >>= 1) {
            if (tid < o) s_d[tid] += s_d[tid + o];
            __syncthreads();
        }
        return s_d[0];
    };
    if (pass == 0) {
        unsigned long long c0 = 0, c1 = 0;
        for (int b = tid; b < nblk; b += 256) {
            c0 += lp->cnt[b][0];
            c1 += lp->cnt[b][1];
        }
        const unsigned long long n0 = block_sum_u64(c0), n1 = block_sum_u64(c1);
        if (tid == 0) {
            const unsigned long long k = n0 < n1 ? n0 : n1;
            stt->cnt[0] = n0;
            stt->cnt[1] = n1;
            stt->k = k;
            s_k = k;
            for (int c = 0; c < 2; ++c) {
                stt->prefix[c] = 0;
                stt->ties[c] = 0;
                stt->sum_gt[c] = 0.0;
                s_need[c] = k;
            }
        }
    } else if (tid == 0) {
        s_need[0] = stt->need[0];
        s_need[1] = stt->need[1];
        s_k = stt->k;
    }
    if (tid < 2) s_bin[tid] = -1;
    __syncthreads();
    double tot = 0.0;
    for (int c = 0; c < 2; ++c) {
        unsigned* h = hist + c * 2048;
        unsigned long long loc = 0;
        for (int j = 0; j < per; ++j) loc += h[nb - 1 - (tid * per + j)];
        const unsigned pfx = pass == 0 ? 0u : stt->prefix[c];
        __syncthreads();
        s_sum[tid] = loc;
        __syncthreads();
        if (tid == 0) {
            unsigned long long run = 0;
            for (int t = 0; t < 256; ++t) {
                const unsigned long long v = s_sum[t];
                s_sum[t] = run;
                run += v;
            }
        }
        __syncthreads();
        const unsigned long long need = s_need[c];
        const unsigned long long before = s_sum[tid];
        if (need > 0 && before < need && before + loc >= need) {
            unsigned long long run = before;
            for (int j = 0; j < per; ++j) {
                const int bin = nb - 1 - (tid * per + j);
                const unsigned long long v = h[bin];
                if (run + v >= need) {
                    stt->prefix[c] = (pfx << (pass == 0 ? 11 : 10)) | (unsigned)bin;
                    stt->need[c] = need - run;
                    stt->ties[c] = v;
                    s_need[c] = need - run;
                    s_ties[c] = v;
                    s_bin[c] = bin;
                    break;
                }
                run += v;
            }
        } else if (need == 0 && tid == 0) {
            stt->need[c] = 0;
        }
        __syncthreads();
        if (pass == 2) {
            const int bin = s_bin[c];
            const unsigned long long ties = bin >= 0 ? s_ties[c] : 0ull, needc = bin >= 0 ? s_need[c] : 0ull;
            const unsigned thr = bin >= 0 ? ((pfx << 10) | (unsigned)bin) : pfx;
            double in_b = 0.0;
            if (bin >= 0)
                for (int j = 0; j < per; ++j) {
                    const int bj = nb - 1 - (tid * per + j);
                    if (bj > bin && h[bj]) in_b += (double)h[bj] * (double)__uint_as_float((pfx << 10) | (unsigned)bj);
                }
            double above = 0.0;
            for (int b = tid; b < nblk; b += 256) above += lp->sum[b][c];
            const double sum_gt = block_sum_f64(above) + block_sum_f64(in_b);
            if (tid == 0) {
                stt->sum_gt[c] = sum_gt;
                stt->frac[c] = ties ? (float)((double)needc / (double)ties) : 0.f;
            }
            tot += sum_gt + (double)needc * (double)__uint_as_float(thr);
        }
        __syncthreads();
    }
    for (int i = tid; i < LOSS_HIST_WORDS; i += 256) hist[i] = 0;
    if (pass == 2 && tid == 0) {
        const unsigned long long k = s_k;
        const float loss = k ? (float)(tot / (2.0 * (double)k)) : __uint_as_float(0x7fc00000u);
        stt->loss = loss;
        stt->inv2k = k ? (float)(1.0 / (2.0 * (double)k)) : 0.f;
        *loss_out = loss;
    }
}

template <int VEC>
__global__ __launch_bounds__(256) void k_bce_bwd(const float* __restrict__ pred, const float* __restrict__ target, const float* __restrict__ lpx,
                                                 const unsigned char* __restrict__ cls, const LossState* __restrict__ stt,
                                                 const float* __restrict__ gout, float* __restrict__ gpred, long P) {
    const unsigned t0 = stt->prefix[0], t1 = stt->prefix[1];
    const float f0 = stt->frac[0], f1 = stt->frac[1];
    const float s = gout[0] * stt->inv2k;
    auto grad = [&](unsigned char c, float l, float p, float tg) -> float {
        if (!c) return 0.f;
        const unsigned key = loss_key(l);
        const unsigned thr = c == 1 ? t0 : t1;
        const float wgt = key > thr ? 1.f : (key == thr ? (c == 1 ? f0 : f1) : 0.f);
        if (wgt == 0.f) return 0.f;
        const float t = fminf(fmaxf(tg, 0.f), 1.f);
        return s * wgt * (p - t) / fmaxf((1.f - p) * p, 1e-12f);
    };
    const long nq = P / VEC;
    for (long q = (long)blockIdx.x * 256 + threadIdx.x; q < nq; q += (long)gridDim.x * 256) {
        const QuadB<VEC> cq = ldqb<VEC>(cls, q);
        const Quad<VEC> lq = ldq<VEC>(lpx, q), pq = ldq<VEC>(pred, q), tq = ldq<VEC>(target, q);
        Quad<VEC> gq;
#pragma unroll
        for (int e = 0; e < VEC; ++e) gq.v[e] = grad(cq.v[e], lq.v[e], pq.v[e], tq.v[e]);
        stq<VEC>(gpred, q, gq);
    }
    if (VEC > 1 && blockIdx.x == 0 && threadIdx.x < P - nq * VEC) {
        const long i = nq * VEC + threadIdx.x;
        gpred[i] = grad(cls[i], lpx[i], pred[i], target[i]);
    }
}

static constexpr int OPT_CHUNK = 2048;

__global__ __launch_bounds__(256) void k_multi_sumsq(const long long* __restrict__ table, const int* __restrict__ chunks,
                                                     double* __restrict__ out) {
    const int t = chunks[2 * blockIdx.x], ch = chunks[2 * blockIdx.x + 1];
    const float* g = reinterpret_cast<const float*>(table[5 * t + 1]);
    const long n = table[5 * t + 4];
    float s = 0.f;
    for (long i = (long)ch * OPT_CHUNK + threadIdx.x; i < n && i < (long)(ch + 1) * OPT_CHUNK; i += 256) s = fmaf(g[i], g[i], s);
    __shared__ float s_w[4];
    s = wave_sum(s);
    if ((threadIdx.x & 63) == 0) s_w[threadIdx.x >> 6] = s;
    __syncthreads();
    if (threadIdx.x == 0) atomicAdd(out, (double)((s_w[0] + s_w[1]) + (s_w[2] + s_w[3])));
}

__global__ void k_clip_coef(const double* sumsq, float max_norm, float* norm_out, float* coef_out) {
    const float norm = (float)sqrt(*sumsq);
    *norm_out = norm;
    *coef_out = fminf(1.f, max_norm / (norm + 1e-6f));
}

__global__ __launch_bounds__(256) void k_multi_scale(const long long* __restrict__ table, const int* __restrict__ chunks,
                                                     const float* __restrict__ coef) {
    const int t = chunks[2 * blockIdx.x], ch = chunks[2 * blockIdx.x + 1];
    float* g = reinterpret_cast<float*>(table[5 * t + 1]);
    const long n = table[5 * t + 4];
    const float c = *coef;
    for (long i = (long)ch * OPT_CHUNK + threadIdx.x; i < n && i < (long)(ch + 1) * OPT_CHUNK; i += 256) g[i] *= c;
}

__global__ __launch_bounds__(256) void k_multi_adam(const long long* __restrict__ table, const int* __restrict__ chunks, float b1, float b2,
                                                    float eps, float step_size, float bc2_sqrt, const float* __restrict__ gscale) {
    const int t = chunks[2 * blockIdx.x], ch = chunks[2 * blockIdx.x + 1];
    float* p = reinterpret_cast<float*>(table[5 * t + 0]);
    const float* g = reinterpret_cast<const float*>(table[5 * t + 1]);
    float* m = reinterpret_cast<float*>(table[5 * t + 2]);
    float* v = reinterpret_cast<float*>(table[5 * t + 3]);
    const long n = table[5 * t + 4];
    const float gs = gscale ? *gscale : 1.f;
    for (long i = (long)ch * OPT_CHUNK + threadIdx.x; i < n && i < (long)(ch + 1) * OPT_CHUNK; i += 256) {
        const float gi = g[i] * gs;
        const float mi = m[i] + (gi - m[i]) * (1.f - b1);
        const float vi = v[i] * b2 + (1.f - b2) * gi * gi;
        m[i] = mi;
        v[i] = vi;
        const float denom = sqrtf(vi) / bc2_sqrt + eps;
        p[i] -= step_size * (mi / denom);
    }
}

__global__ void k_step_inc(float* step) { *step += 1.f; }
__global__ __launch_bounds__(256) void k_multi_adam_dev(const long long* __restrict__ table, const int* __restrict__ chunks, double b1d, double b2d,
                                                        float eps, double lr, const float* __restrict__ step, const float* __restrict__ gscale) {
    const float b1 = (float)b1d, b2 = (float)b2d;
    const int t = chunks[2 * blockIdx.x], ch = chunks[2 * blockIdx.x + 1];
    float* p = reinterpret_cast<float*>(table[5 * t + 0]);
    const float* g = reinterpret_cast<const float*>(table[5 * t + 1]);
    float* m = reinterpret_cast<float*>(table[5 * t + 2]);
    float* v = reinterpret_cast<float*>(table[5 * t + 3]);
    const long n = table[5 * t + 4];
    const double st = (double)*step;
    const float step_size = (float)(lr / (1.0 - pow(b1d, st)));
    const float bc2_sqrt = (float)sqrt(1.0 - pow(b2d, st));
    const float gs = gscale ? *gscale : 1.f;
    for (long i = (long)ch * OPT_CHUNK + threadIdx.x; i < n && i < (long)(ch + 1) * OPT_CHUNK; i += 256) {
        const float gi = g[i] * gs;
        const float mi = m[i] + (gi - m[i]) * (1.f - b1);
        const float vi = v[i] * b2 + (1.f - b2) * gi * gi;
        m[i] = mi;
        v[i] = vi;
        const float denom = sqrtf(vi) / bc2_sqrt + eps;
        p[i] -= step_size * (mi / denom);
    }
}

__global__ void k_fill_f32(float* p, float v, long n) {
    for (long i = (long)blockIdx.x * 256 + threadIdx.x; i < n; i += (long)gridDim.x * 256) p[i] = v;
}

__global__ void k_fold64_multi(const int* __restrict__ table, float* __restrict__ dst, const double* __restrict__ src) {
    const int d = table[blockIdx.x * 3], s0 = table[blockIdx.x * 3 + 1], n = table[blockIdx.x * 3 + 2];
    for (int i = threadIdx.x; i < n; i += 64) dst[d + i] = (float)((double)dst[d + i] + src[s0 + i]);
}

extern "C" {

long ocrs_loss_state_bytes() { return (long)sizeof(LossState); }
long ocrs_loss_hist_bytes() { return LOSS_HIST_WORDS * (long)sizeof(unsigned) + (long)sizeof(LossParts); }

int ocrs_balanced_bce_fwd(const float* pred, const float* target, float* lpx, unsigned char* cls, void* state, void* hist, float* loss_out,
                          long P, hipStream_t st) {
    OCRS_CHECK_ARG(pred && target && lpx && cls && state && hist && loss_out && P > 0);
    LossState* stt = (LossState*)state;
    if (hipMemsetAsync(hist, 0, LOSS_HIST_WORDS * sizeof(unsigned), st) != hipSuccess) return OCRS_ERR_HIP;
    int grid = ew_grid((P + 3) / 4);
    if (grid > LOSS_MAXB) grid = LOSS_MAXB;
    const bool vec = ((reinterpret_cast<uintptr_t>(pred) | reinterpret_cast<uintptr_t>(target) | reinterpret_cast<uintptr_t>(lpx)) & 15) == 0 &&
                     (reinterpret_cast<uintptr_t>(cls) & 3) == 0;
    if (vec)
        hipLaunchKernelGGL(k_bce_fwd<4>, dim3(grid), dim3(256), 0, st, pred, target, lpx, cls, (unsigned*)hist, P);
    else
        hipLaunchKernelGGL(k_bce_fwd<1>, dim3(grid), dim3(256), 0, st, pred, target, lpx, cls, (unsigned*)hist, P);
    for (int pass = 0; pass < 3; ++pass) {
        if (pass > 0) {
            if (vec)
                hipLaunchKernelGGL(k_select_hist<4>, dim3(grid), dim3(256), 0, st, lpx, cls, stt, (unsigned*)hist, pass, P);
            else
                hipLaunchKernelGGL(k_select_hist<1>, dim3(grid), dim3(256), 0, st, lpx, cls, stt, (unsigned*)hist, pass, P);
        }
        hipLaunchKernelGGL(k_select_scan, dim3(1), dim3(256), 0, st, stt, (unsigned*)hist, pass, grid, loss_out);
    }
    OCRS_LAUNCH_CHECK();
    return OCRS_OK;
}

int ocrs_balanced_bce_bwd(const float* pred, const float* target, const float* lpx, const unsigned char* cls, const void* state,
                          const float* gout, float* gpred, long P, hipStream_t st) {
    OCRS_CHECK_ARG(pred && target && lpx && cls && state && gout && gpred && P > 0);
    const bool vec = ((reinterpret_cast<uintptr_t>(pred) | reinterpret_cast<uintptr_t>(target) | reinterpret_cast<uintptr_t>(lpx) |
                       reinterpret_cast<uintptr_t>(gpred)) & 15) == 0 && (reinterpret_cast<uintptr_t>(cls) & 3) == 0;
    if (vec)
        hipLaunchKernelGGL(k_bce_bwd<4>, dim3(ew_grid((P + 3) / 4)), dim3(256), 0, st, pred, target, lpx, cls, (const LossState*)state, gout, gpred, P);
    else
        hipLaunchKernelGGL(k_bce_bwd<1>, dim3(ew_grid(P)), dim3(256), 0, st, pred, target, lpx, cls, (const LossState*)state, gout, gpred, P);
    OCRS_LAUNCH_CHECK();
    return OCRS_OK;
}

int ocrs_opt_chunk() { return OPT_CHUNK; }

int ocrs_clip_grad_norm(const long long* table, const int* chunks, int nchunks, float max_norm, double* sumsq, float* norm_out,
                        float* coef_out, int scale_in_place, hipStream_t st) {
    OCRS_CHECK_ARG(table && chunks && nchunks > 0 && sumsq && norm_out && coef_out);
    if (hipMemsetAsync(sumsq, 0, sizeof(double), st) != hipSuccess) return OCRS_ERR_HIP;
    hipLaunchKernelGGL(k_multi_sumsq, dim3(nchunks), dim3(256), 0, st, table, chunks, sumsq);
    hipLaunchKernelGGL(k_clip_coef, dim3(1), dim3(1), 0, st, sumsq, max_norm, norm_out, coef_out);
    if (scale_in_place) hipLaunchKernelGGL(k_multi_scale, dim3(nchunks), dim3(256), 0, st, table, chunks, coef_out);
    OCRS_LAUNCH_CHECK();
    return OCRS_OK;
}

int ocrs_adam_step(const long long* table, const int* chunks, int nchunks, float b1, float b2, float eps, float step_size, float bc2_sqrt,
                   const float* gscale, hipStream_t st) {
    OCRS_CHECK_ARG(table && chunks && nchunks > 0);
    hipLaunchKernelGGL(k_multi_adam, dim3(nchunks), dim3(256), 0, st, table, chunks, b1, b2, eps, step_size, bc2_sqrt, gscale);
    OCRS_LAUNCH_CHECK();
    return OCRS_OK;
}

int ocrs_adam_step_dev(const long long* table, const int* chunks, int nchunks, double b1, double b2, float eps, double lr, float* step,
                       const float* gscale, hipStream_t st) {
    OCRS_CHECK_ARG(table && chunks && nchunks > 0 && step);
    hipLaunchKernelGGL(k_step_inc, dim3(1), dim3(1), 0, st, step);
    hipLaunchKernelGGL(k_multi_adam_dev, dim3(nchunks), dim3(256), 0, st, table, chunks, b1, b2, eps, lr, step, gscale);
    OCRS_LAUNCH_CHECK();
    return OCRS_OK;
}

int ocrs_fold64_multi(const int* table, int nrows, float* dst, const double* src, hipStream_t st) {
    OCRS_CHECK_ARG(table && nrows > 0 && dst && src);
    hipLaunchKernelGGL(k_fold64_multi, dim3(nrows), dim3(64), 0, st, table, dst, src);
    OCRS_LAUNCH_CHECK();
    return OCRS_OK;
}

int ocrs_fill_f32(float* p, float v, long n, hipStream_t st) {
    OCRS_CHECK_ARG(p && n >= 0);
    if (n == 0) return OCRS_OK;
    hipLaunchKernelGGL(k_fill_f32, dim3(ew_grid(n)), dim3(256), 0, st, p, v, n);
    OCRS_LAUNCH_CHECK();
    return OCRS_OK;
}

}
```

ocrs_models_amd/csrc/loss_state.h:

```cpp
#pragma once
struct LossState {
    unsigned long long cnt[2];
    unsigned long long k;
    unsigned prefix[2];
    unsigned long long need[2];
    unsigned long long ties[2];
    double sum_gt[2];
    float loss;
    float frac[2];
    float inv2k;
};

__device__ __forceinline__ unsigned loss_key(float v) { return __float_as_uint(v) & 0x7fffffffu; }
```

ocrs_models_amd/ddp.py:

```python
from __future__ import annotations

import os

import torch
import torch.distributed as dist
from torch import nn


class GradBucketer:
    def __init__(self, process_group=None, bucket_bytes: int = 1 << 20, average: bool = True):
        self.pg = process_group
        self.bucket_bytes = int(os.environ.get("OCRS_DDP_BUCKET_BYTES", bucket_bytes))
        self.average = average
        self.world = dist.get_world_size(process_group) if dist.is_initialized() else 1
        self.force = bool(int(os.environ.get("OCRS_DDP_FORCE", "0"))) and dist.is_initialized()
        self._reset()

    def _reset(self):
        self._pending_lo = None
        self._pending_hi = None
        self._works = []
        self.launched = []

    timing = None

    def exposed_ms(self):
        return [e0.elapsed_time(e1) for e0, e1 in (self.timing or [])]

    def ready(self, flat: torch.Tensor, lo: int, hi: int):
        if self._pending_lo is None:
            self._pending_lo, self._pending_hi = lo, hi
        else:
            if lo != self._pending_hi:
                raise RuntimeError(f"non-contiguous gradient range: expected {self._pending_hi}, got {lo}")
            self._pending_hi = hi
        if (self._pending_hi - self._pending_lo) * flat.element_size() >= self.bucket_bytes:
            self._launch(flat)

    def _launch(self, flat):
        lo, hi = self._pending_lo, self._pending_hi
        self._pending_lo = self._pending_hi = None
        if hi <= lo:
            return
        self.launched.append((lo, hi))
        if self.world == 1 and not self.force:
            return
        chunk = flat[lo:hi]
        if self.average:
            chunk.mul_(1.0 / self.world)
        self._works.append(dist.all_reduce(chunk, op=dist.ReduceOp.SUM, group=self.pg, async_op=True))

    def finish(self, flat: torch.Tensor):
        if self._pending_lo is not None:
            self._launch(flat)
        ev = None
        if self.timing is not None and flat.is_cuda and self._works:
            ev = (torch.cuda.Event(enable_timing=True), torch.cuda.Event(enable_timing=True))
            ev[0].record()
        for w in self._works:
            w.wait()
        if ev is not None:
            ev[1].record()
            self.timing.append(ev)
        ranges = self.launched
        self.last_ranges = ranges
        self._reset()
        return ranges


class DistributedDataParallel(nn.Module):

    def __init__(self, module: nn.Module, process_group=None, bucket_bytes: int = 1 << 20, broadcast_buffers: bool = False):
        super().__init__()
        self.module = module
        self.pg = process_group
        self.broadcast_buffers = broadcast_buffers
        self.bucketer = GradBucketer(process_group, bucket_bytes)
        if dist.is_initialized() and dist.get_world_size(process_group) > 1:
            with torch.no_grad():
                for t in list(module.parameters()) + list(module.buffers()):
                    dist.broadcast(t, src=0, group=process_group)
        module._grad_bucketer = self.bucketer

    def forward(self, *args, **kwargs):
        if self.broadcast_buffers and dist.is_initialized() and dist.get_world_size(self.pg) > 1:
            with torch.no_grad():
                for b in self.module.buffers():
                    dist.broadcast(b, src=0, group=self.pg)
        return self.module(*args, **kwargs)

    def state_dict(self, *a, **k):
        return self.module.state_dict(*a, **k)

    def load_state_dict(self, *a, **k):
        return self.module.load_state_dict(*a, **k)
```

ocrs_models_amd/losses.py:

```python
from __future__ import annotations

import contextlib

import torch

from ._lib import lib, ptr


_FUSE = {"on": False}
_PENDING = {}
_ZERO = {}


@contextlib.contextmanager
def fused_head_backward():
    prev, _FUSE["on"] = _FUSE["on"], True
    try:
        yield
    except BaseException:
        _FUSE["on"] = prev
        if not prev:
            _PENDING.clear()
        raise
    else:
        _FUSE["on"] = prev
        if not prev and _PENDING:
            _PENDING.clear()
            raise RuntimeError("fused_head_backward(): a deferred loss gradient was never consumed by a DetectionModel backward")


def _zero_marker(dev):
    z = _ZERO.get(dev.index)
    if z is None:
        z = _ZERO[dev.index] = torch.zeros(1, dtype=torch.float32, device=dev)
    return z


def take_deferred(gpred: torch.Tensor, pred: torch.Tensor):
    z = _ZERO.get(gpred.device.index)
    is_marker = z is not None and gpred.data_ptr() == z.data_ptr() and all(s == 0 for s in gpred.stride())
    saved = _PENDING.pop((gpred.device.index, pred.data_ptr()), None)
    if saved is None:
        if is_marker:
            raise RuntimeError("fused_head_backward(): the network's backward received the deferred-gradient marker but no loss gradient is parked "
                               "for its prediction tensor")
        return None, False
    return saved, is_marker


def materialize_deferred(saved) -> torch.Tensor:
    pred, target, lpx, cls, state, g = saved
    gpred = torch.empty_like(pred)
    lib().balanced_bce_bwd(ptr(pred), ptr(target), ptr(lpx), ptr(cls), ptr(state), ptr(g), ptr(gpred), pred.numel())
    return gpred


class _BalancedBCE(torch.autograd.Function):
    @staticmethod
    def forward(ctx, pred, target):
        L = lib()
        ctx.from_det = type(pred.grad_fn).__name__ == "_DetFnBackward" and pred.is_contiguous() and pred.dtype == torch.float32
        pred = pred.contiguous().float()
        target = target.contiguous().float()
        P = pred.numel()
        dev = pred.device
        lpx = torch.empty(P, dtype=torch.float32, device=dev)
        cls = torch.empty(P, dtype=torch.uint8, device=dev)
        state = torch.empty(L.loss_state_bytes(), dtype=torch.uint8, device=dev)
        hist = torch.empty(L.loss_hist_bytes(), dtype=torch.uint8, device=dev)
        loss = torch.empty((), dtype=torch.float32, device=dev)
        L.balanced_bce_fwd(ptr(pred), ptr(target), ptr(lpx), ptr(cls), ptr(state), ptr(hist), ptr(loss), P)
        ctx.save_for_backward(pred, target, lpx, cls, state)
        return loss

    @staticmethod
    def backward(ctx, gout):
        pred, target, lpx, cls, state = ctx.saved_tensors
        g = gout.contiguous().float().reshape(1)
        key = (pred.device.index, pred.data_ptr())
        if _FUSE["on"] and ctx.from_det and key not in _PENDING:
            _PENDING[key] = (pred, target, lpx, cls, state, g)
            return _zero_marker(pred.device).expand(pred.shape), None
        gpred = torch.empty_like(pred)
        lib().balanced_bce_bwd(ptr(pred), ptr(target), ptr(lpx), ptr(cls), ptr(state), ptr(g), ptr(gpred), pred.numel())
        return gpred, None


def balanced_cross_entropy_loss(pred: torch.Tensor, target: torch.Tensor) -> torch.Tensor:
    if not pred.is_cuda:
        raise RuntimeError("ocrs_models_amd losses run on MI355X only (no CPU path)")
    if pred.shape != target.shape:
        raise RuntimeError(f"pred {tuple(pred.shape)} and target {tuple(target.shape)} must have the same shape")
    return _BalancedBCE.apply(pred, target)


MAX_CTC_STATES = 4096


_CTC_AB = True


class _CTC(torch.autograd.Function):
    @staticmethod
    def forward(ctx, log_probs, targets, in_len, tg_len, smax=None, h16=False):
        L = lib()
        lp = log_probs.contiguous().float()
        T, N, C = lp.shape
        tg = targets.contiguous().to(torch.int32)
        Lpad = tg.shape[1]
        Smax = smax or 2 * Lpad + 1
        dev = lp.device
        nll = torch.empty(N, dtype=torch.float32, device=dev)
        loss = torch.empty((), dtype=torch.float32, device=dev)
        ctx.ab = False
        if h16:
            alpha = torch.empty(N, T, Smax, dtype=torch.float16, device=dev)
            rowmax = torch.empty(N, T, dtype=torch.float32, device=dev)
            L.ctc_fwd_h16(ptr(lp), ptr(tg), ptr(in_len), ptr(tg_len), ptr(alpha), ptr(rowmax), ptr(nll), ptr(loss), T, N, C, Lpad, Smax)
        else:
            alpha = torch.empty(N, T, Smax, dtype=torch.float32, device=dev)
            rowmax = nll
            if ctx.needs_input_grad[0] and _CTC_AB:
                rowmax = torch.empty(N, T, Smax, dtype=torch.float32, device=dev)
                L.ctc_fwd_ab(ptr(lp), ptr(tg), ptr(in_len), ptr(tg_len), ptr(alpha), ptr(rowmax), ptr(nll), ptr(loss), T, N, C, Lpad, Smax)
                ctx.ab = True
            else:
                L.ctc_fwd(ptr(lp), ptr(tg), ptr(in_len), ptr(tg_len), ptr(alpha), ptr(nll), ptr(loss), T, N, C, Lpad, Smax)
        ctx.save_for_backward(lp, tg, in_len, tg_len, alpha, nll, rowmax)
        ctx.smax, ctx.h16 = Smax, h16
        return loss

    @staticmethod
    def backward(ctx, gout):
        lp, tg, in_len, tg_len, alpha, nll, rowmax = ctx.saved_tensors
        T, N, C = lp.shape
        grad = torch.empty_like(lp)
        g = gout.contiguous().float().reshape(1)
        if ctx.ab:
            lib().ctc_grad_ab(ptr(lp), ptr(tg), ptr(in_len), ptr(tg_len), ptr(alpha), ptr(rowmax), ptr(nll), ptr(g), ptr(grad), T, N, C, tg.shape[1], ctx.smax)
        elif ctx.h16:
            lib().ctc_bwd_h16(ptr(lp), ptr(tg), ptr(in_len), ptr(tg_len), ptr(alpha), ptr(rowmax), ptr(nll), ptr(g), ptr(grad), T, N, C, tg.shape[1], ctx.smax)
        else:
            lib().ctc_bwd(ptr(lp), ptr(tg), ptr(in_len), ptr(tg_len), ptr(alpha), ptr(nll), ptr(g), ptr(grad), T, N, C, tg.shape[1], ctx.smax)
        return grad, None, None, None, None, None


class CTCLoss(torch.nn.Module):

    def __init__(self, blank: int = 0, reduction: str = "mean", zero_infinity: bool = False, lattice_dtype: torch.dtype = torch.float32):
        super().__init__()
        if blank != 0 or reduction != "mean" or zero_infinity:
            raise NotImplementedError("only torch.nn.CTCLoss() defaults are implemented (the reference's configuration)")
        if lattice_dtype not in (torch.float32, torch.float16):
            raise ValueError("lattice_dtype must be torch.float32 or torch.float16")
        self.h16 = lattice_dtype == torch.float16

    def forward(self, log_probs, targets, input_lengths, target_lengths):
        if not log_probs.is_cuda:
            raise RuntimeError("ocrs_models_amd losses run on MI355X only (no CPU path)")
        if targets.dim() != 2:
            raise RuntimeError("targets must be (N, Lpad) padded label rows (the layout collate_samples produces)")
        dev = log_probs.device
        il = torch.as_tensor(input_lengths, dtype=torch.int64)
        tl = torch.as_tensor(target_lengths, dtype=torch.int64)
        T, N = log_probs.shape[0], log_probs.shape[1]
        smax = None
        if il.shape != (N,) or tl.shape != (N,) or targets.shape[0] != N:
            raise RuntimeError(f"input_lengths / target_lengths / targets must have batch size {N}")
        if not il.is_cuda and not tl.is_cuda and N > 0:
            if int(il.max()) > T or int(il.min()) < 0:
                raise RuntimeError(f"Expected input_lengths to have value at most {T}, but got value {int(il.max())} (while checking arguments for ctc_loss)")
            if int(tl.max()) > targets.shape[1] or int(tl.min()) < 0:
                raise RuntimeError(f"Expected tensor to have size at least {int(tl.max())} at dimension 1, but got size {tuple(targets.shape)} "
                                   "(while checking arguments for ctc_loss)")
            smax = 2 * int(tl.max()) + 1
        if (smax or 2 * targets.shape[1] + 1) > MAX_CTC_STATES:
            raise RuntimeError(f"CTC lattices wider than {MAX_CTC_STATES} states (targets longer than {(MAX_CTC_STATES - 1) // 2} labels) are not "
                               "supported by the LDS-resident alpha/beta kernels; pass host-side target_lengths so that the padding does not count")
        if not il.is_cuda and not tl.is_cuda:
            both = torch.stack([il, tl]).to(dev, non_blocking=True)
            il, tl = both[0], both[1]
        return _CTC.apply(log_probs, targets.to(dev), il.to(dev, non_blocking=True), tl.to(dev, non_blocking=True), smax, self.h16)
```

ocrs_models_amd/models.py:

```python
from __future__ import annotations

import math

import torch
from torch import nn

from ._lib import DT, lib, ptr
from .packs import EMPTY as EMPTY_PACKS, PackRow, cached_table, dgrad_row, fwd_row

DEPTH_SCALE = [8, 16, 32, 32, 64, 128, 256]
_DT = DT


class DepthwiseConv(nn.Module):

    def __init__(self, in_channels: int, out_channels: int):
        super().__init__()
        self.seq = nn.Sequential(
            nn.Conv2d(in_channels, in_channels, 3, padding=1, bias=False, groups=in_channels),
            nn.Conv2d(in_channels, out_channels, 1, bias=False),
            nn.BatchNorm2d(out_channels),
            nn.ReLU(),
        )


class DoubleConv(nn.Module):
    def __init__(self, in_channels: int, out_channels: int):
        super().__init__()
        self.seq = nn.Sequential(DepthwiseConv(in_channels, out_channels), DepthwiseConv(out_channels, out_channels))


class Down(nn.Module):
    def __init__(self, in_channels: int, out_channels: int):
        super().__init__()
        self.seq = nn.Sequential(DoubleConv(in_channels, out_channels), nn.MaxPool2d(2))


class Up(nn.Module):
    def __init__(self, in_up_channels: int, in_cross_channels: int, out_channels: int):
        super().__init__()
        self.up = nn.ConvTranspose2d(in_up_channels, out_channels, kernel_size=3, stride=2)
        self.contract = DoubleConv(out_channels + in_cross_channels, out_channels)


class _Act:

    __slots__ = ("t", "tr", "C", "H", "W", "src", "other_use", "u", "wexp")

    def __init__(self, t, tr, C, H, W, src=None):
        self.t, self.tr, self.C, self.H, self.W = t, tr, C, H, W
        self.u = self.wexp = None
        self.src, self.other_use = src, False


class _BlockRec:

    __slots__ = ("prefix", "a", "b", "z", "tr", "saved", "Cin", "Cout", "H", "W", "fsum")

    def __init__(self, prefix, a, b, z, tr, saved, Cin, Cout, H, W, fsum=None):
        self.prefix, self.a, self.b, self.z, self.tr, self.saved = prefix, a, b, z, tr, saved
        self.Cin, self.Cout, self.H, self.W, self.fsum = Cin, Cout, H, W, fsum


def _srcs(a, b):
    if b is None:
        return ptr(a.t), None, a.C, 0, ptr(a.tr), None
    return ptr(a.t), ptr(b.t), a.C, b.C, ptr(a.tr), ptr(b.tr)


_identity_cache: dict = {}


def _identity_tr(C, device):
    key = (C, device)
    t = _identity_cache.get(key)
    if t is None:
        t = torch.empty(3, C, dtype=torch.float32, device=device)
        t[0] = 1.0
        t[1] = 0.0
        t[2] = -math.inf
        _identity_cache[key] = t
    return t


class _DetRun:

    overlap = True
    use_mm = use_rs32 = fuse_bn_bwd = fold_fwd_fin = True
    c1_u = c1_noz = c1_fuse = head_gl = True
    packs = EMPTY_PACKS
    _zpool, _zoff = None, 0
    _flat, _folds, _defer_folds = None, (), False
    _keep_ws, _deferring = None, False
    _head_gl = _c1acc = None

    def __init__(self, P, Bf, dev, dtype, N, train=True, mod=None, x=None):
        self.L = lib()
        self.P, self.Bf, self.names = P, Bf, list(P)
        self.dev, self.dtype, self.dt, self.N, self.train = dev, dtype, DT[dtype], N, train
        self.mod, self.x = mod, x
        self.recs = {}
        self.fused = {}
        self.pooled_by_block = None
        self.capture = getattr(mod, "_capture", None)
        if self.capture is not None:
            self.capture["run"] = self

    def empty(self, *shape, dtype=None):
        return torch.empty(shape, dtype=dtype or self.dtype, device=self.dev)

    def fits32(self, H, W, C):
        return self.N * H * W * C * 4 < 2 ** 32

    def bn_fin(self, prefix, C):
        P, Bf = self.P, self.Bf
        tr, saved = self.empty(3, C, dtype=torch.float32), self.empty(2, C, dtype=torch.float32)
        return tr, saved, (ptr(P[f"{prefix}.weight"]), ptr(P[f"{prefix}.bias"]), 1e-5, 0.1, ptr(tr), ptr(saved), ptr(Bf[f"{prefix}.running_mean"]),
                           ptr(Bf[f"{prefix}.running_var"]), ptr(Bf[f"{prefix}.num_batches_tracked"]), 0.0)

    def _hold(self, ws):
        if self._keep_ws is not None:
            self._keep_ws.append(ws)

    def zeros64(self, n):
        pool = self._zpool
        n8 = (n + 7) // 8 * 8
        if pool is None or self._zoff + n8 > pool.numel():
            if pool is not None and self._folds and self.overlap:
                torch.cuda.current_stream().wait_stream(_side_stream(self.dev))
            self.fold_flush()
            pool = self._zpool = torch.zeros(max(8192, n8), dtype=torch.float64, device=self.dev)
            self._zoff = 0
        out = pool[self._zoff:self._zoff + n]
        self._zoff += n8
        return out

    def fold64(self, dst, src64):
        if self._flat is None or not self._defer_folds or src64._base is not self._zpool:
            dst.view(-1).add_(src64)
            return
        self._folds.append((dst.storage_offset(), src64.storage_offset(), src64.numel()))

    _FOLD_TABLES = {}

    def fold_flush(self):
        folds = self._folds
        if not folds:
            return
        key = (self.dev, tuple(folds))
        tab = _DetRun._FOLD_TABLES.get(key)
        if tab is None:
            if len(_DetRun._FOLD_TABLES) > 64:
                _DetRun._FOLD_TABLES.clear()
            tab = _DetRun._FOLD_TABLES[key] = torch.tensor(folds, dtype=torch.int32).to(self.dev)
        self.L.fold64_multi(ptr(tab), len(folds), ptr(self._flat), ptr(self._zpool))
        folds.clear()

    def pack(self, src, mode, K, M, K2, s1, s2, sm):
        return self.packs.fetch(PackRow(src, self.dt, mode, K, M, K2, s1, s2, sm), self.dev)

    def convt_row(self, w):
        Cup, Cout = w.shape[0], w.shape[1]
        return PackRow(w, self.dt, 1, 4 * Cup, 4 * Cout, Cup, 0, 0, 0)

    def convt_dgrad_row(self, w):
        Cup, Cout = w.shape[0], w.shape[1]
        return PackRow(w, self.dt, 0, 9 * Cout, Cup, Cout, 1, 9, 9 * Cout)

    def pack_rows(self):
        P, rows = self.P, []
        for name in self.names:
            if name.endswith(".seq.1.weight") and P[name].dim() == 4 and P[name].shape[1] > 1:
                rows += [fwd_row(P[name], self.dt), dgrad_row(P[name], self.dt)]
        for i in range(6):
            rows += [self.convt_row(P[f"up.{i}.up.weight"]), self.convt_dgrad_row(P[f"up.{i}.up.weight"])]
        return rows

    def prepack(self):
        key = (self.dt, tuple(p.data_ptr() for p in self.P.values()))
        self.packs = cached_table(self.mod, key, self.pack_rows, self.dev)
        self.packs.launch()

    def bn_tr(self, prefix, gstat, count, C, nparts=0):
        P, Bf = self.P, self.Bf
        tr, saved, fin = self.bn_fin(prefix, C)
        if self.train and nparts:
            self.L.bn_finalize_parts(ptr(gstat), nparts, count, C, *fin)
        elif self.train:
            self.L.bn_finalize(ptr(gstat), count, C, *fin)
        else:
            rstd = torch.rsqrt(Bf[f"{prefix}.running_var"] + 1e-5)
            tr[0] = P[f"{prefix}.weight"].detach() * rstd
            tr[1] = P[f"{prefix}.bias"].detach() - Bf[f"{prefix}.running_mean"] * tr[0]
            tr[2] = 0.0
        return tr, saved

    def fwd_route(self, Ca, Cb, Cout, H, W):
        if self.use_mm and self.L.mm_fwd_supported(Ca, Cb, Cout, self.dt):
            return "mm"
        if self.use_rs32 and self.L.rs32_fwd_supported(Ca, Cb, Cout, self.dt) and self.fits32(H, W, max(Ca + Cb, Cout)):
            return "rs32"
        return "tile"

    def bwd_route(self, r, pooled, need_gx):
        if r.Cin == 1:
            return "c1"
        L, C, H, W = self.L, r.Cout, r.H, r.W
        Ca, Cb = r.a.C, (r.b.C if r.b is not None else 0)
        if self.use_mm and need_gx and H >= 2 and W >= 2 and L.mm_bwd_supported(Ca, Cb, C, self.dt):
            return "mm"
        if (self.use_rs32 and need_gx and L.rs32_bwd_supported(Ca, Cb, C, 1 if pooled else 0, self.dt) and self.fits32(H, W, max(r.Cin, C))
                and (not pooled or (H >= 2 and W >= 2))):
            return "rs32"
        return "tile"

    def block(self, prefix, a, b, Cout, pool=False):
        L, P, N = self.L, self.P, self.N
        H, W = a.H, a.W
        Cb = b.C if b is not None else 0
        Cin = a.C + Cb
        wdw, wpw = P[f"{prefix}.seq.0.weight"], P[f"{prefix}.seq.1.weight"]
        z = self.empty(N, H, W, Cout)
        bnp = f"{prefix}.seq.2"
        fin = self.train and self.fold_fwd_fin
        pooled = gamma = None
        route = self.fwd_route(a.C, Cb, Cout, H, W)
        if route == "mm":
            if pool:
                pooled, gamma = self.empty(N, H // 2, W // 2, Cout), P[f"{bnp}.weight"]
            nparts = L.mm_fwd_nparts(a.C, Cb, Cout, N, H, W)
            parts = self.empty(nparts * 2 * Cout, dtype=torch.float32)
            if fin and a.u is not None and b is None and pooled is None and Cout in (8, 16):
                tr, saved, fin_args = self.bn_fin(bnp, Cout)
                L.mm_fwd_fin_xu(ptr(a.u), ptr(a.wexp), ptr(a.tr), ptr(wdw), ptr(wpw), ptr(z), ptr(parts), ptr(self.zeros64(1)), N * H * W, *fin_args,
                                Cout, N, H, W, self.dt)
            elif fin:
                tr, saved, fin_args = self.bn_fin(bnp, Cout)
                L.mm_fwd_fin(*_srcs(a, b), ptr(wdw), ptr(wpw), ptr(z), ptr(parts), ptr(gamma), ptr(pooled), ptr(self.zeros64(1)), N * H * W, *fin_args,
                             Cout, N, H, W, self.dt)
            else:
                L.mm_fwd(*_srcs(a, b), ptr(wdw), ptr(wpw), ptr(z), ptr(parts), ptr(gamma), ptr(pooled), Cout, N, H, W, self.dt)
                tr, saved = self.bn_tr(bnp, parts, N * H * W, Cout, nparts=nparts)
        elif route == "rs32":
            if pool:
                pooled, gamma = self.empty(N, H // 2, W // 2, Cout), P[f"{bnp}.weight"]
            gstat = self.zeros64(2 * Cout)
            common = (*_srcs(a, b), ptr(wdw), ptr(wpw), ptr(z), ptr(gstat), ptr(gamma), ptr(pooled))
            if fin:
                tr, saved, fin_args = self.bn_fin(bnp, Cout)
                L.rs32_fwd(*common, ptr(self.zeros64(1)), N * H * W, *fin_args, Cout, N, H, W)
            else:
                L.rs32_fwd(*common, None, 0, None, None, 0.0, 0.0, None, None, None, None, None, 0.0, Cout, N, H, W)
                tr, saved = self.bn_tr(bnp, gstat, N * H * W, Cout)
        else:
            wpk = self.packs.fetch(fwd_row(wpw, self.dt), self.dev)
            gstat = self.zeros64(2 * Cout)
            if pool and L.dwpw_fwd_pool_supported(Cin, Cout):
                pooled, gamma = self.empty(N, H // 2, W // 2, Cout), P[f"{bnp}.weight"]
            if fin and pooled is None and L.dwpw_fwd_fin_supported(Cin, Cout, self.dt):
                tr, saved, fin_args = self.bn_fin(bnp, Cout)
                L.dwpw_fwd_fin(*_srcs(a, b), ptr(wdw), ptr(wpk), ptr(z), ptr(gstat), ptr(self.zeros64(1)), N * H * W, *fin_args, Cout, N, H, W, self.dt)
            else:
                L.dwpw_fwd(*_srcs(a, b), ptr(wdw), ptr(wpk), ptr(z), ptr(gstat), ptr(gamma), ptr(pooled), Cout, N, H, W, self.dt)
                tr, saved = self.bn_tr(bnp, gstat, N * H * W, Cout)
        self.pooled_by_block = pooled
        self.recs[prefix] = _BlockRec(prefix, a, b, z, tr, saved, Cin, Cout, H, W)
        return _Act(z, tr, Cout, H, W, src=prefix)

    def block_c1(self, prefix, img, H, W):
        L, P, N = self.L, self.P, self.N
        wdw, wpw = P[f"{prefix}.seq.0.weight"], P[f"{prefix}.seq.1.weight"]
        z = self.empty(N, H, W, 8)
        gstat = self.zeros64(16)
        uplane = fsum = None
        if self.train and self.c1_u and self.use_mm and L.dwpw_c1_u_supported(N, H, W, self.dt):
            uplane = torch.empty(N, H, W, dtype=torch.bfloat16, device=self.dev)
            if (self.c1_noz and self.capture is None and self.fold_fwd_fin and self.fuse_bn_bwd and L.mm_fwd_supported(8, 0, 8, self.dt)
                    and L.mm_bwd_head_supported(8, 0, 8, N, H, W, self.dt)):
                z = None
            fsum = self.zeros64(20) if (z is None and self.c1_fuse) else None
            if fsum is not None:
                L.dwpw_c1_fwd_us(ptr(img), ptr(wdw), ptr(wpw), ptr(z), ptr(uplane), ptr(gstat), ptr(fsum), N, H, W, self.dt)
            else:
                L.dwpw_c1_fwd_u(ptr(img), ptr(wdw), ptr(wpw), ptr(z), ptr(uplane), ptr(gstat), N, H, W, self.dt)
        else:
            L.dwpw_c1_fwd(ptr(img), ptr(wdw), ptr(wpw), ptr(z), ptr(gstat), N, H, W, self.dt)
        tr, saved = self.bn_tr(f"{prefix}.seq.2", gstat, N * H * W, 8)
        self.recs[prefix] = _BlockRec(prefix, None, None, z, tr, saved, 1, 8, H, W, fsum)
        out = _Act(z, tr, 8, H, W, src=prefix)
        out.u, out.wexp = uplane, wpw
        return out

    def double(self, prefix, a, b, Cout, pool=False):
        y = self.block(f"{prefix}.seq.0", a, b, Cout)
        return self.block(f"{prefix}.seq.1", y, None, Cout, pool=pool)

    def forward(self):
        L, P, N, w = self.L, self.P, self.N, DEPTH_SCALE
        x = self.x
        H, W = x.shape[2], x.shape[3]
        if H < 64 or W < 64:
            raise RuntimeError(f"DetectionModel needs H, W >= 64 (six 2x2 poolings), got {H}x{W}")
        self.prepack()
        a0 = self.block_c1("in_conv.seq.0", x, H, W)
        cur = self.block("in_conv.seq.1", a0, None, w[0])
        skips = [cur]
        for i in range(6):
            y = self.double(f"down.{i}.seq.0", cur, None, w[i + 1], pool=True)
            Hp, Wp = y.H // 2, y.W // 2
            pooled = self.pooled_by_block
            y.other_use = True
            if pooled is None:
                pooled = self.empty(N, Hp, Wp, y.C)
                L.maxpool_fwd(ptr(y.t), ptr(y.tr), ptr(pooled), y.C, N, y.H, y.W, 1, self.dt)
            cur = _Act(pooled, y.tr, y.C, Hp, Wp, src=y.src)
            skips.append(cur)
        up = skips[6]
        self.convt = {}
        for i in reversed(range(6)):
            skip = skips[i]
            Cup, Cout = w[i + 1], w[i]
            wpk = self.packs.fetch(self.convt_row(P[f"up.{i}.up.weight"]), self.dev)
            t = self.empty(N, skip.H, skip.W, Cout)
            up.other_use = True
            if self.use_rs32 and L.rs32_convt_fwd_supported(Cup, Cout, self.dt) and self.fits32(skip.H, skip.W, Cout):
                L.rs32_convt_fwd(ptr(up.t), ptr(up.tr), ptr(P[f"up.{i}.up.weight"]), ptr(P[f"up.{i}.up.bias"]), ptr(t), Cup, Cout, N, up.H, up.W, skip.H, skip.W)
            else:
                L.convt_fwd(ptr(up.t), ptr(up.tr), ptr(wpk), ptr(P[f"up.{i}.up.bias"]), ptr(t), Cup, Cout, N, up.H, up.W, skip.H, skip.W, self.dt)
            ta = _Act(t, _identity_tr(Cout, self.dev), Cout, skip.H, skip.W)
            self.convt[i] = (up, ta)
            up = self.double(f"up.{i}.contract", ta, skip, Cout)
        pred = self.empty(N, 1, H, W, dtype=torch.float32)
        up.other_use = True
        L.head_fwd(ptr(up.t), ptr(up.tr), ptr(P["out_conv.0.weight"]), ptr(P["out_conv.0.bias"]), ptr(pred), N * H * W, self.dt)
        self.head_in, self.pred, self.skips, self.HW = up, pred, skips, (H, W)
        return pred

    def block_bwd(self, prefix, g1, g2, pooled, need_gx=True):
        gxa, gxb = self._block_bwd(prefix, g1, g2, pooled, need_gx)
        if self.capture is not None:
            self.capture[prefix] = {"g1": g1, "g2": g2, "pooled": pooled, "gxa": gxa, "gxb": gxb}
        return gxa, gxb

    def _block_bwd(self, prefix, g1, g2, pooled, need_gx=True):
        L, P, N, r = self.L, self.P, self.N, self.recs[prefix]
        C, H, W = r.Cout, r.H, r.W
        gsum = self.fused.pop(prefix, None)
        if gsum is None:
            gsum = self.zeros64(2 * C)
            L.bn_bwd_reduce(ptr(g1), ptr(g2), pooled, ptr(r.z), ptr(r.tr), ptr(r.saved), ptr(gsum), C, N, H, W, self.dt)
        route = self.bwd_route(r, pooled, need_gx)
        gam, wdw, wpw = P[f"{prefix}.seq.2.weight"], P[f"{prefix}.seq.0.weight"], P[f"{prefix}.seq.1.weight"]
        dWdw, dWpw, dgamma, dbeta = (self.G[f"{prefix}.seq.{k}"] for k in ("0.weight", "1.weight", "2.weight", "2.bias"))
        if route == "c1":
            coef = self.empty(3, C, dtype=torch.float32)
            L.bn_bwd_finalize(ptr(gsum), N * H * W, C, ptr(gam), ptr(r.saved), ptr(coef), ptr(dgamma), ptr(dbeta))
            acc = self.zeros64(17)
            if self._c1acc is not None:
                c1acc, self._c1acc = self._c1acc, None
                L.c1_bwd_fin(ptr(c1acc), ptr(r.fsum), ptr(coef), ptr(wpw), ptr(acc))
            else:
                L.dwpw_c1_bwd(ptr(self.x), ptr(wdw), ptr(wpw), ptr(g1), ptr(g2), pooled, ptr(r.z), ptr(r.tr), ptr(coef), ptr(acc), N, H, W, self.dt)
            self.fold64(dWpw, acc[:8])
            self.fold64(dWdw, acc[8:17])
            return None, None
        a, b = r.a, r.b
        Ca, Cb = a.C, (b.C if b is not None else 0)
        wpk_d = self.packs.fetch(dgrad_row(wpw, self.dt), self.dev)

        def stat_target(act):
            if act is None or act.src is None or act.other_use or not need_gx or not self.fuse_bn_bwd:
                return None, None
            if act.src not in self.fused:
                self.fused[act.src] = self.zeros64(2 * act.C)
            return self.recs[act.src].saved, self.fused[act.src]
        if route in ("mm", "rs32"):
            gxa = self.empty(N, H, W, Ca)
            gxb = self.empty(N, H, W, Cb) if b is not None else None
            sva, gsa = stat_target(a)
            svb, gsb = stat_target(b)
            ws = self.empty((L.mm_bwd_ws_floats if route == "mm" else L.rs32_bwd_ws_floats)(Ca, Cb, C, N, H, W), dtype=torch.float32)
            self._hold(ws)
            if self._head_gl is not None and g1 is self._head_gl:
                head = (ptr(a.t), Ca, ptr(a.tr), ptr(wdw), ptr(wpw), ptr(g1), ptr(P["out_conv.0.weight"]), ptr(r.z), ptr(r.tr), ptr(gsum), ptr(gam),
                        ptr(r.saved), ptr(dgamma), ptr(dbeta), ptr(gxa), ptr(dWpw), ptr(dWdw), ptr(ws), ptr(sva), ptr(gsa), C, N, H, W)
                self._head_gl = None
                if route == "mm":
                    L.mm_bwd_fin_head(*head, self.dt)
                else:
                    L.rs32_bwd_head(*head)
                return gxa, gxb
            if route == "rs32":
                L.rs32_bwd(*_srcs(a, b), ptr(wdw), ptr(wpw), ptr(g1), ptr(g2), ptr(r.z), ptr(r.tr), ptr(gsum), ptr(gam), ptr(r.saved), ptr(dgamma),
                           ptr(dbeta), ptr(gxa), ptr(gxb), ptr(dWpw), ptr(dWdw), ptr(ws), ptr(sva), ptr(gsa), ptr(svb), ptr(gsb), 1 if pooled else 0,
                           C, N, H, W)
                return gxa, gxb
            if a.u is not None and b is None and not pooled and L.mm_bwd_head_supported(Ca, 0, C, N, H, W, self.dt):
                r1 = self.recs.get(a.src) if a.src is not None else None
                if r1 is not None and r1.fsum is not None and C == 8 and sva is not None and self.capture is None:
                    c1acc = self.zeros64(8 * 32)
                    L.mm_bwd_fin_xu_c1(ptr(a.u), ptr(a.wexp), ptr(a.tr), ptr(wdw), ptr(wpw), ptr(g1), ptr(g2), ptr(r.z), ptr(r.tr), ptr(gsum), ptr(gam),
                                       ptr(r.saved), ptr(dgamma), ptr(dbeta), ptr(dWpw), ptr(dWdw), ptr(ws), ptr(sva), ptr(gsa), ptr(self.x), ptr(c1acc),
                                       C, N, H, W, self.dt)
                    self._c1acc = c1acc
                    return None, None
                L.mm_bwd_fin_xu(ptr(a.u), ptr(a.wexp), ptr(a.tr), ptr(wdw), ptr(wpw), ptr(g1), ptr(g2), ptr(r.z), ptr(r.tr), ptr(gsum), ptr(gam), ptr(r.saved),
                                ptr(dgamma), ptr(dbeta), ptr(gxa), ptr(dWpw), ptr(dWdw), ptr(ws), ptr(sva), ptr(gsa), C, N, H, W, self.dt)
                return gxa, gxb
            L.mm_bwd_fin(*_srcs(a, b), ptr(wdw), ptr(wpw), ptr(g1), ptr(g2), pooled, ptr(r.z), ptr(r.tr), ptr(gsum), ptr(gam), ptr(r.saved), ptr(dgamma),
                         ptr(dbeta), ptr(gxa), ptr(gxb), ptr(dWpw), ptr(dWdw), ptr(ws), ptr(sva), ptr(gsa), ptr(svb), ptr(gsb), C, N, H, W, self.dt)
            return gxa, gxb
        coef = self.empty(3, C, dtype=torch.float32)
        du = self.empty(N, H, W, r.Cin)
        ws = self.empty(L.pw_bwd_ws_floats(r.Cin, C, N, H, W), dtype=torch.float32)
        self._hold(ws)
        L.pw_bwd_fin(*_srcs(a, b), ptr(wdw), ptr(g1), ptr(g2), pooled, ptr(r.z), ptr(r.tr), ptr(coef), ptr(gsum), ptr(gam), ptr(r.saved), ptr(dgamma),
                     ptr(dbeta), ptr(wpk_d), ptr(du), ptr(dWpw), ptr(ws), C, N, H, W, self.dt)
        gxa = self.empty(N, H, W, Ca) if need_gx else None
        gxb = self.empty(N, H, W, Cb) if (need_gx and b is not None) else None
        ws = self.empty(L.dw_bwd_ws_floats(r.Cin, N, H, W), dtype=torch.float32)
        self._hold(ws)
        sva, gsa = stat_target(a)
        svb, gsb = stat_target(b)
        L.dw_bwd(*_srcs(a, b), ptr(wdw), ptr(du), ptr(gxa), ptr(gxb), ptr(dWdw), ptr(ws), ptr(sva), ptr(gsa), ptr(svb), ptr(gsb), N, H, W, self.dt)
        return gxa, gxb

    def backward(self, gpred):
        self._deferring = False
        try:
            return self._backward(gpred)
        finally:
            if self._deferring:
                self._deferring = False
                self.L.bwd_defer_flush()
            self._keep_ws = None

    def _backward(self, gpred):
        L, P, N, w = self.L, self.P, self.N, DEPTH_SCALE
        H, W = self.HW
        flat = torch.zeros(sum(p.numel() for p in P.values()), dtype=torch.float32, device=self.dev)
        order = ["out_conv"] + [f"up.{i}" for i in range(6)] + [f"down.{i}" for i in reversed(range(6))] + ["in_conv"]
        self.G, off, stage_end = {}, 0, {}
        for stage in order:
            for k in self.names:
                if k.startswith(stage + "."):
                    n = P[k].numel()
                    self.G[k] = flat[off:off + n].view_as(P[k])
                    off += n
            stage_end[stage] = off
        bucketer = getattr(self.mod, "_grad_bucketer", None)
        self._flat, self._folds = flat, []
        self._defer_folds = bucketer is None and self.capture is None
        self._keep_ws = []
        if bucketer is None and self.capture is None:
            scratch = _bwd_scratch(self.dev)
            L.bwd_defer_begin(ptr(scratch), scratch.numel())
            self._deferring = True
        done = [0]
        main = torch.cuda.current_stream()
        side = _side_stream(self.dev) if self.overlap else None
        pending, keep = [], []

        def stage_done(stage, side_work=False):
            if side_work:
                pending.append(stage)
                return
            if bucketer is not None:
                bucketer.ready(flat, done[0], stage_end[stage])
            done[0] = stage_end[stage]

        def flush_pending():
            if pending:
                main.wait_stream(side)
                for st in pending:
                    stage_done(st)
                pending.clear()
                keep.clear()
        from . import losses as _losses
        deferred, is_marker = _losses.take_deferred(gpred, self.pred)
        if deferred is not None and not is_marker:
            gpred = gpred + _losses.materialize_deferred(deferred)
            deferred = None
        gpred = gpred.contiguous().float() if deferred is None else None
        up = self.head_in
        sv = gs_head = None
        if self.fuse_bn_bwd and up.src is not None:
            sv, gs_head = self.recs[up.src].saved, self.zeros64(16)
            self.fused[up.src] = gs_head
        acc = self.zeros64(9)
        r_up = self.recs[up.src] if gs_head is not None else None
        head_gl = False
        if self.head_gl and self.capture is None and r_up is not None and r_up.b is None:
            route = self.bwd_route(r_up, 0, True)
            head_gl = bool((route == "mm" and L.mm_bwd_head_supported(r_up.a.C, 0, r_up.Cout, N, H, W, self.dt))
                           or (route == "rs32" and L.rs32_bwd_head_supported(r_up.a.C, 0, r_up.Cout, self.dt)))
        if deferred is not None and not (head_gl and (N * H * W) % 4 == 0 and deferred[0].data_ptr() == self.pred.data_ptr()):
            gpred, deferred = _losses.materialize_deferred(deferred), None
        if deferred is not None:
            g = self.empty(N, H, W, dtype=torch.float32)
            _, d_target, d_lpx, d_cls, d_state, d_gout = deferred
            L.head_bwd_loss(ptr(up.t), ptr(up.tr), ptr(P["out_conv.0.weight"]), ptr(self.pred), ptr(d_target), ptr(d_lpx), ptr(d_cls), ptr(d_state),
                            ptr(d_gout), ptr(g), ptr(acc), ptr(sv), ptr(gs_head), N * H * W, self.dt)
        elif head_gl:
            g = self.empty(N, H, W, dtype=torch.float32)
            L.head_bwd_gl(ptr(up.t), ptr(up.tr), ptr(P["out_conv.0.weight"]), ptr(self.pred), ptr(gpred), ptr(g), ptr(acc), ptr(sv), ptr(gs_head),
                          N * H * W, self.dt)
        else:
            g = self.empty(N, H, W, 8)
            L.head_bwd(ptr(up.t), ptr(up.tr), ptr(P["out_conv.0.weight"]), ptr(self.pred), ptr(gpred), ptr(g), ptr(acc), ptr(sv), ptr(gs_head),
                       N * H * W, self.dt)
        self._head_gl = g if head_gl else None
        self.fold64(self.G["out_conv.0.weight"], acc[:8])
        self.fold64(self.G["out_conv.0.bias"], acc[8:9])
        if self.capture is not None:
            self.capture["out_conv"] = {"gpred": gpred, "g": g}
        stage_done("out_conv")
        skip_g = [[] for _ in range(7)]
        for i in range(6):
            g1, _ = self.block_bwd(f"up.{i}.contract.seq.1", g, None, 0)
            if bucketer is not None:
                flush_pending()
            gxa, gxb = self.block_bwd(f"up.{i}.contract.seq.0", g1, None, 0)
            skip_g[i].append(gxb)
            up_in, ta = self.convt[i]
            Cup, Cout = w[i + 1], w[i]
            wpk_d = self.packs.fetch(self.convt_dgrad_row(P[f"up.{i}.up.weight"]), self.dev)
            dx = self.empty(N, up_in.H, up_in.W, Cup)
            ws = self.empty(L.convt_bwd_ws_floats(Cup, Cout, N, up_in.H, up_in.W, self.dt), dtype=torch.float32)
            self._hold(ws)
            sv = gs_up = None
            rs_ctd = (self.use_rs32 and L.rs32_convt_dgrad_supported(Cup, Cout, self.dt) and self.fits32(ta.H, ta.W, Cout)
                      and L.convt_bwd_splittable(Cup, Cout, self.dt))
            if self.fuse_bn_bwd and up_in.src is not None and (rs_ctd or L.convt_bwd_stats_supported(Cup, Cout, self.dt)):
                sv, gs_up = self.recs[up_in.src].saved, self.zeros64(2 * Cup)
                self.fused[up_in.src] = gs_up
            db64 = self.zeros64(Cout)
            args = (ptr(up_in.t), ptr(up_in.tr), ptr(gxa), ptr(wpk_d), ptr(dx), ptr(self.G[f"up.{i}.up.weight"]), ptr(self.G[f"up.{i}.up.bias"]), ptr(db64),
                    ptr(ws), None if rs_ctd else ptr(sv), None if rs_ctd else ptr(gs_up), Cup, Cout, N, up_in.H, up_in.W, ta.H, ta.W)

            def dgrad():
                if rs_ctd:
                    L.rs32_convt_dgrad(ptr(gxa), ptr(P[f"up.{i}.up.weight"]), ptr(dx), ptr(up_in.t), ptr(up_in.tr), ptr(sv), ptr(gs_up), Cup, Cout, N,
                                       up_in.H, up_in.W, ta.H, ta.W)
                else:
                    L.convt_bwd_parts(*args, 1, self.dt)
            if side is not None and L.convt_bwd_splittable(Cup, Cout, self.dt):
                flush_pending()
                side.wait_stream(main)
                with torch.cuda.stream(side):
                    L.convt_bwd_parts(*args, 2, self.dt)
                    if not self._defer_folds:
                        self.G[f"up.{i}.up.bias"].add_(db64)
                if self._defer_folds:
                    self.fold64(self.G[f"up.{i}.up.bias"], db64)
                keep.extend((gxa, ws, db64, wpk_d, up_in.t))
                dgrad()
                stage_done(f"up.{i}", side_work=True)
            else:
                flush_pending()
                if rs_ctd:
                    L.convt_bwd_parts(*args, 2, self.dt)
                    dgrad()
                else:
                    L.convt_bwd(*args, self.dt)
                self.fold64(self.G[f"up.{i}.up.bias"], db64)
                stage_done(f"up.{i}")
            if self.capture is not None:
                self.capture[f"up.{i}.up"] = {"g": gxa, "dx": dx}
            g = dx
        skip_g[6].append(g)
        for i in reversed(range(6)):
            gs = skip_g[i + 1]
            g1, _ = self.block_bwd(f"down.{i}.seq.0.seq.1", gs[0], gs[1] if len(gs) > 1 else None, 1)
            if bucketer is not None:
                flush_pending()
            gx, _ = self.block_bwd(f"down.{i}.seq.0.seq.0", g1, None, 0)
            stage_done(f"down.{i}")
            skip_g[i].append(gx)
        gs = skip_g[0]
        g1, _ = self.block_bwd("in_conv.seq.1", gs[0], gs[1], 0)
        self.block_bwd("in_conv.seq.0", g1, None, 0)
        flush_pending()
        if side is not None and self._defer_folds:
            main.wait_stream(side)
        if self._deferring:
            self._deferring = False
            L.bwd_defer_flush()
        self.fold_flush()
        self._flat = None
        stage_done("in_conv")
        if bucketer is not None:
            bucketer.finish(flat)
        if self.capture is not None:
            self.capture["grads"] = dict(self.G)
        return [self.G[k] for k in self.names]


_SIDE = {}
_BWD_SCRATCH = {}


def _bwd_scratch(dev):
    t = _BWD_SCRATCH.get(dev)
    if t is None:
        t = _BWD_SCRATCH[dev] = torch.zeros(65536, dtype=torch.float64, device=dev)
    return t


def _side_stream(dev):
    st = _SIDE.get(dev)
    if st is None:
        st = _SIDE[dev] = torch.cuda.Stream(device=dev)
    return st


def _check_versions(ctx):
    if ctx.run is None:
        raise RuntimeError("Trying to backward through the graph a second time: the saved activations of this network were freed by the first "
                           "backward (retain_graph is not supported by the fused whole-network autograd node)")
    for p, v in zip(ctx.params, ctx.versions):
        if p._version != v:
            raise RuntimeError("one of the parameters needed for gradient computation has been modified by an inplace operation "
                               "(e.g. optimizer.step()) between forward and backward")


class _DetFn(torch.autograd.Function):
    @staticmethod
    def forward(ctx, run, *params):
        pred = run.forward()
        ctx.run = run
        ctx.params = params
        ctx.versions = [p._version for p in params]
        return pred

    @staticmethod
    def backward(ctx, gpred):
        _check_versions(ctx)
        grads = ctx.run.backward(gpred)
        ctx.run = None
        return (None, *grads)


class DetectionModel(nn.Module):

    def __init__(self, act_dtype: torch.dtype | None = None):
        super().__init__()
        depth_scale = DEPTH_SCALE
        self.depth_scale = depth_scale
        self.in_conv = DoubleConv(1, depth_scale[0])
        self.down = nn.ModuleList(Down(depth_scale[i], depth_scale[i + 1]) for i in range(len(depth_scale) - 1))
        self.up = nn.ModuleList(Up(depth_scale[i + 1], depth_scale[i], depth_scale[i]) for i in range(len(depth_scale) - 1))
        self.out_conv = nn.Sequential(nn.Conv2d(depth_scale[0], 1, kernel_size=1), nn.Sigmoid())
        self.act_dtype = act_dtype

    def _act_dtype(self):
        if self.act_dtype is not None:
            return self.act_dtype
        if torch.is_autocast_enabled("cuda") and torch.get_autocast_dtype("cuda") == torch.bfloat16:
            return torch.bfloat16
        return torch.float32

    def forward(self, x: torch.Tensor) -> torch.Tensor:
        if not x.is_cuda:
            raise RuntimeError("ocrs_models_amd.DetectionModel runs on MI355X only (no CPU path); move the model and input to 'cuda'")
        if x.dim() != 4 or x.shape[1] != 1:
            raise RuntimeError(f"expected (B,1,H,W) input, got {tuple(x.shape)}")
        x = x.contiguous().float()
        names = [n for n, _ in self.named_parameters()]
        params = [p for _, p in self.named_parameters()]
        for p in params:
            if p.dtype != torch.float32 or not p.is_contiguous():
                raise RuntimeError("parameters must be contiguous fp32")
        run = _DetRun(dict(zip(names, (p.detach() for p in params))), dict(self.named_buffers()), x.device, self._act_dtype(), x.shape[0],
                      self.training, mod=self, x=x)
        if torch.is_grad_enabled() and any(p.requires_grad for p in params):
            return _DetFn.apply(run, *params)
        return run.forward()
```

ocrs_models_amd/train_detection.py:

```python
from __future__ import annotations

import os
import shutil
from argparse import ArgumentParser, BooleanOptionalAction

import torch

from .checkpoint import load_checkpoint, save_checkpoint
from .losses import balanced_cross_entropy_loss, fused_head_backward
from .models import DetectionModel
from .optim import Adam


def make_optimizer(model: DetectionModel) -> Adam:
    return Adam(model.parameters())


def train_step(model, optimizer, batch: dict, device, loss_fn=balanced_cross_entropy_loss) -> torch.Tensor:
    img = batch["image"].to(device, non_blocking=True)
    masks = batch["text_mask"].to(device, non_blocking=True)
    pred_masks = model(img)
    loss = loss_fn(pred_masks, masks)
    optimizer.zero_grad()
    if loss_fn is balanced_cross_entropy_loss:
        with fused_head_backward():
            loss.backward()
    else:
        loss.backward()
    optimizer.step()
    return loss.detach()


def train(epoch: int, device, dataloader, model, loss_fn, optimizer) -> float:
    model.train()
    total = torch.zeros((), device=device)
    n = 0
    for batch in dataloader:
        total += train_step(model, optimizer, batch, device, loss_fn)
        n += 1
    return float(total.item()) / max(n, 1)


def binarize_mask(mask: torch.Tensor, threshold: float = 0.5) -> torch.Tensor:
    return torch.where(mask > threshold, 1.0, 0.0)


def mean(values: list[float]) -> float:
    return sum(values) / len(values)


def get_metric_means(metrics_dicts: list[dict[str, float]]) -> dict[str, float]:
    if not len(metrics_dicts):
        return {}
    keys = set(k for md in metrics_dicts for k in md.keys())
    return {k: mean([md.get(k, 0.0) for md in metrics_dicts]) for k in keys}


def test(device, dataloader, model, loss_fn=balanced_cross_entropy_loss, metrics_fn="default") -> tuple[float, dict[str, float]]:
    device_metrics = isinstance(metrics_fn, str) and metrics_fn == "device"
    if isinstance(metrics_fn, str) and metrics_fn == "default":
        from .postprocess import mask_metrics as metrics_fn
    elif device_metrics:
        from .postprocess import METRIC_KEYS, batch_mask_metrics
    model.eval()
    n_batches = 0
    n_images = 0
    metrics = []
    with torch.inference_mode():
        total = torch.zeros((), device=device)
        msum = torch.zeros(4, dtype=torch.float64, device=device) if device_metrics else None
        for batch in dataloader:
            img = batch["image"].to(device, non_blocking=True)
            masks = batch["text_mask"].to(device, non_blocking=True)
            pred_masks = model(img)
            total += loss_fn(pred_masks, masks)
            n_batches += 1
            if device_metrics:
                msum += batch_mask_metrics(pred_masks, masks).sum(0)
                n_images += pred_masks.shape[0]
            elif metrics_fn is not None:
                bin_pred_masks = binarize_mask(pred_masks).cpu()
                bin_masks = binarize_mask(masks).cpu()
                for item_index, bin_pred_mask in enumerate(bin_pred_masks):
                    metrics.append(metrics_fn(bin_pred_mask, bin_masks[item_index]))
    if device_metrics:
        vals = torch.cat([total.double().reshape(1), msum]).tolist()
        return vals[0] / max(n_batches, 1), ({k: v / n_images for k, v in zip(METRIC_KEYS, vals[1:])} if n_images else {})
    return float(total.item()) / max(n_batches, 1), get_metric_means(metrics)


def format_metrics(metrics: dict[str, float]) -> dict[str, str]:
    return {k: f"{v:.3f}" for k, v in metrics.items()}


def save_img_and_predicted_mask(basename: str, img_filename: str, img: torch.Tensor, pred_masks, target_masks=None):
    from PIL import Image

    def to_pil(t):
        return Image.fromarray(t.detach().float().mul(255).byte().cpu().numpy().reshape(t.shape[-2:]), "L")

    shutil.copyfile(img_filename, f"{basename}_input.png")
    to_pil(img + 0.5).save(f"{basename}_input_scaled.png")
    for i, pred_mask in enumerate(pred_masks):
        to_pil(pred_mask).save(f"{basename}_pred_mask_{i}.png")
    if target_masks is not None:
        for i, target_mask in enumerate(target_masks):
            to_pil(target_mask).save(f"{basename}_mask_{i}.png")


class _DebugImages:

    def __init__(self, loader, model, basename: str):
        self.loader, self.model, self.basename = loader, model, basename

    def __len__(self):
        return len(self.loader)

    def __iter__(self):
        for batch in self.loader:
            yield batch
            was_training = self.model.training
            self.model.eval()
            with torch.no_grad():
                pred = self.model(batch["image"][:1])
            self.model.train(was_training)
            save_img_and_predicted_mask(self.basename, batch["path"][0], batch["image"][0], pred[0], [batch["text_mask"][0]])


CHECKPOINT_FILE = "text-detection-checkpoint.pt"


def prepare_loaders(dataset_type: str, data_dir: str, batch_size: int, max_images=None, augment=True, device="cuda", mask_size=None):
    from .datasets import DDI100, DevicePageLoader, HierText

    if dataset_type == "ddi":
        load_dataset = DDI100
    elif dataset_type == "hiertext":
        load_dataset = HierText
    else:
        raise Exception(f"Unknown dataset type {dataset_type}")
    validation_max_images = max(10, int(max_images * 0.1)) if max_images else None
    train_dataset = load_dataset(data_dir, augment=augment, train=True, max_images=max_images, device=device, mask_size=mask_size)
    train_dataloader = DevicePageLoader(train_dataset, batch_size=batch_size, shuffle=True)
    val_dataset = load_dataset(data_dir, augment=augment, train=False, max_images=validation_max_images, device=device, mask_size=mask_size)
    val_dataloader = DevicePageLoader(val_dataset, batch_size=batch_size)
    return train_dataset, train_dataloader, val_dataset, val_dataloader


def main(argv=None):
    parser = ArgumentParser(description="Train text detection model.")
    parser.add_argument("dataset_type", type=str, choices=["ddi", "hiertext"], help="Format of dataset")
    parser.add_argument("data_dir")
    parser.add_argument("--batch-size", type=int, default=4, help="Batch size")
    parser.add_argument("--checkpoint", type=str, help="Model checkpoint to load")
    parser.add_argument("--debug-images", action="store_true", help="Save debugging images during training")
    parser.add_argument("--export", type=str, help="Export model to ONNX format")
    parser.add_argument("--max-epochs", type=int, help="Maximum number of epochs to train for")
    parser.add_argument("--max-images", type=int, help="Maximum number of images to load")
    parser.add_argument("--validate-only", action="store_true", help="Run validation on an existing model")
    parser.add_argument("--augment", default=True, action=BooleanOptionalAction, help="Enable data augmentation")
    args = parser.parse_args(argv)

    if not torch.cuda.is_available():
        raise RuntimeError("ocrs_models_amd.train_detection runs on MI355X only (no CPU path)")
    torch.manual_seed(1234)
    device = torch.device("cuda", torch.cuda.current_device())

    train_dataset, train_dataloader, val_dataset, val_dataloader = prepare_loaders(args.dataset_type, args.data_dir, args.batch_size,
                                                                                   args.max_images, args.augment, device)
    print(f"Training dataset: images {len(train_dataset)} in {len(train_dataloader)} batches")
    print(f"Validation dataset: images {len(val_dataset)} in {len(val_dataloader)} batches")

    model = DetectionModel().to(device)
    optimizer = make_optimizer(model)
    total_params = sum(p.numel() for p in model.parameters() if p.requires_grad)
    print(f"Model param count: {total_params}")

    epochs_without_improvement = 0
    min_train_loss = 1.0
    epoch = 0
    if args.checkpoint:
        checkpoint = load_checkpoint(args.checkpoint, model, optimizer, device)
        epoch = checkpoint["epoch"]

    if args.export:
        if not args.checkpoint:
            raise Exception("ONNX export requires a checkpoint to load")
        import importlib.util

        if importlib.util.find_spec("onnx") is None:
            parser.exit(1, "--export needs the onnx package, which is not installed\n")
        from .export import export_onnx

        test_batch = next(iter(val_dataloader))
        export_onnx(model, args.export, test_batch["image"][0:1].to(device))
        return

    train_loader, val_loader = train_dataloader, val_dataloader
    if args.debug_images:
        train_loader = _DebugImages(train_dataloader, model, "train-sample")
        val_loader = _DebugImages(val_dataloader, model, "test-sample")

    if args.validate_only:
        if not args.checkpoint:
            parser.exit(1, "Existing model should be specified with --checkpoint when using --validate-only")
        val_loss, val_metrics = test(device, val_loader, model, balanced_cross_entropy_loss, metrics_fn="device")
        print(f"Validation loss {val_loss:.4f}")
        print("Validation metrics:", format_metrics(val_metrics))
        return

    while args.max_epochs is None or epoch < args.max_epochs:
        train_loss = train(epoch, device, train_loader, model, balanced_cross_entropy_loss, optimizer)
        val_loss, val_metrics = test(device, val_loader, model, balanced_cross_entropy_loss, metrics_fn="device")
        print(f"Epoch {epoch} train loss {train_loss:.4f} validation loss {val_loss:.4f}")
        print(f"Epoch {epoch} validation metrics:", format_metrics(val_metrics))
        if train_loss < min_train_loss:
            min_train_loss = train_loss
            epochs_without_improvement = 0
            save_checkpoint(CHECKPOINT_FILE, model, optimizer, epoch=epoch)
        else:
            epochs_without_improvement += 1
        if epochs_without_improvement > 3:
            print(f"Stopping after {epochs_without_improvement} epochs without train loss improvement")
        epoch += 1


if __name__ == "__main__":
    main()
```

Measured before the change: 2704.

## Fuse detection head forward with balanced BCE loss pass and streamline select scan

Adds a kernel that computes the sigmoid head output and the per-pixel BCE loss, class labels and loss histogram in one pass, so pred no longer has to be written and re-read by a separate loss kernel. The model gains a forward_loss path, and the train step uses it when the default loss is selected. The select-scan kernel is also rewritten to use wave-level shuffle scans and register-held histogram bins in place of shared-memory serial reductions. The cost is extra plumbing through autograd, the DDP wrapper and the model, plus alignment and size preconditions for the fused path.

Result: no change. 2715, median of 6 (+0.4%).

```diff
diff --git a/include/ocrs_hip.h b/include/ocrs_hip.h
--- a/include/ocrs_hip.h
+++ b/include/ocrs_hip.h
@@ -64,6 +64,8 @@
 int ocrs_rs32_convt_dgrad(const float* g, const float* wt, float* dx, const float* x, const float* tr, const float* saved, double* gsum, int Cup, int Cout, int N,
                           int h, int w, int H, int W, hipStream_t st);
 int ocrs_head_fwd(const void* z, const float* tr, const float* w, const float* b, float* pred, long P, int dtype, hipStream_t st);
+int ocrs_head_fwd_loss(const void* z, const float* tr, const float* w, const float* b, const float* target, float* pred, float* lpx,
+                       unsigned char* cls, void* state, void* hist, float* loss_out, long P, int dtype, hipStream_t st);
 
 int ocrs_bn_bwd_reduce(const void* g1, const void* g2, int pooled, const void* z, const float* bn, const float* saved, double* gsum, int C,
                        int N, int H, int W, int dtype, hipStream_t st);
@@ -130,6 +132,7 @@
                           long P, hipStream_t st);
 int ocrs_balanced_bce_bwd(const float* pred, const float* target, const float* lpx, const unsigned char* cls, const void* state,
                           const float* gout, float* gpred, long P, hipStream_t st);
+int ocrs_select_scan(void* state, void* hist, int pass, int nblk, float* loss_out, hipStream_t st);
 int ocrs_fold64_multi(const int* table, int nrows, float* dst, const double* src, hipStream_t st);
 
 int ocrs_conv_igemm(const void* x, int ldx, const void* wpk, void* out, int ldo, const float* bias, int relu, double* gstat, int Cin, int M, int N,
diff --git a/ocrs_models_amd/csrc/det_common.h b/ocrs_models_amd/csrc/det_common.h
--- a/ocrs_models_amd/csrc/det_common.h
+++ b/ocrs_models_amd/csrc/det_common.h
@@ -170,6 +170,14 @@
 __device__ __forceinline__ void apply_tr8(float (&v)[8], const float* tr, int C, int c0) {
 #pragma unroll
     for (int i = 0; i < 8; ++i) v[i] = fmaxf(fmaf(v[i], tr[c0 + i], tr[C + c0 + i]), tr[2 * C + c0 + i]);
+}
+
+__device__ __forceinline__ float head_prob(const float (&v)[8], const float (&wv)[8], const float (&sc)[8], const float (&sh)[8], const float (&lo)[8],
+                                           float bias) {
+    float s = bias;
+#pragma unroll
+    for (int i = 0; i < 8; ++i) s = fmaf(wv[i], fmaxf(fmaf(v[i], sc[i], sh[i]), lo[i]), s);
+    return 1.f / (1.f + __expf(-s));
 }
 
 template <int CG>
diff --git a/ocrs_models_amd/csrc/det_head.hip b/ocrs_models_amd/csrc/det_head.hip
--- a/ocrs_models_amd/csrc/det_head.hip
+++ b/ocrs_models_amd/csrc/det_head.hip
@@ -16,11 +16,53 @@
     for (long p = (long)blockIdx.x * 256 + threadIdx.x; p < P; p += (long)gridDim.x * 256) {
         float v[8];
         load8(z + p * 8, v);
-        float s = bias;
-#pragma unroll
-        for (int i = 0; i < 8; ++i) s = fmaf(wv[i], fmaxf(fmaf(v[i], sc[i], sh[i]), lo[i]), s);
-        pred[p] = 1.f / (1.f + __expf(-s));
-    }
+        pred[p] = head_prob(v, wv, sc, sh, lo, bias);
+    }
+}
+
+template <class T>
+__global__ __launch_bounds__(256) void k_head_fwd_loss(const T* __restrict__ z, const float* __restrict__ tr, const float* __restrict__ w,
+                                                       const float* __restrict__ b, const float* __restrict__ target, float* __restrict__ pred,
+                                                       float* __restrict__ lpx, unsigned char* __restrict__ cls, unsigned* __restrict__ hist, long P) {
+    __shared__ unsigned s_h[LOSS_HIST_WORDS];
+    __shared__ unsigned s_cnt[2];
+    for (int i = threadIdx.x; i < LOSS_HIST_WORDS; i += 256) s_h[i] = 0;
+    __syncthreads();
+    float wv[8], sc[8], sh[8], lo[8];
+#pragma unroll
+    for (int i = 0; i < 8; ++i) {
+        wv[i] = w[i];
+        sc[i] = tr[i];
+        sh[i] = tr[8 + i];
+        lo[i] = tr[16 + i];
+    }
+    const float bias = b[0];
+    unsigned long long np = 0, nn = 0;
+    const long nq = P >> 2;
+    for (long q = (long)blockIdx.x * 256 + threadIdx.x; q < nq; q += (long)gridDim.x * 256) {
+        const float4 t4 = reinterpret_cast<const float4*>(target)[q];
+        float v[4][8];
+#pragma unroll
+        for (int e = 0; e < 4; ++e) load8(z + (q * 4 + e) * 8, v[e]);
+        const float te[4] = {t4.x, t4.y, t4.z, t4.w};
+        float pe[4], le[4];
+        unsigned ce[4];
+#pragma unroll
+        for (int e = 0; e < 4; ++e) {
+            pe[e] = head_prob(v[e], wv, sc, sh, lo, bias);
+            ce[e] = bce_class(te[e]);
+            le[e] = bce_pixel(pe[e], te[e]);
+            np += ce[e] == 1;
+            nn += ce[e] == 2;
+        }
+        reinterpret_cast<float4*>(pred)[q] = make_float4(pe[0], pe[1], pe[2], pe[3]);
+        reinterpret_cast<float4*>(lpx)[q] = make_float4(le[0], le[1], le[2], le[3]);
+        reinterpret_cast<unsigned*>(cls)[q] = ce[0] | (ce[1] << 8) | (ce[2] << 16) | (ce[3] << 24);
+#pragma unroll
+        for (int e = 0; e < 4; ++e)
+            if (ce[e]) atomicAdd(&s_h[(ce[e] - 1) * 2048 + (loss_key(le[e]) >> 20)], 1u);
+    }
+    bce_block_finish(np, nn, s_h, s_cnt, hist);
 }
 
 template <class T>
@@ -176,6 +218,20 @@
     return OCRS_OK;
 }
 
+int ocrs_head_fwd_loss(const void* z, const float* tr, const float* w, const float* b, const float* target, float* pred, float* lpx,
+                       unsigned char* cls, void* state, void* hist, float* loss_out, long P, int dtype, hipStream_t st) {
+    OCRS_CHECK_ARG(z && tr && w && b && target && pred && lpx && cls && state && hist && loss_out && P > 0 && P % 4 == 0);
+    OCRS_CHECK_ARG(aligned16(z) && aligned16(target) && aligned16(pred) && aligned16(lpx) && aligned16(cls) && aligned16(hist));
+    if (hipMemsetAsync(hist, 0, LOSS_HIST_WORDS * sizeof(unsigned), st) != hipSuccess) return OCRS_ERR_HIP;
+    int grid = ew_grid(P / 4);
+    if (grid > LOSS_MAXB) grid = LOSS_MAXB;
+    if (dtype == 1)
+        hipLaunchKernelGGL(k_head_fwd_loss<bf16>, dim3(grid), dim3(256), 0, st, (const bf16*)z, tr, w, b, target, pred, lpx, cls, (unsigned*)hist, P);
+    else
+        hipLaunchKernelGGL(k_head_fwd_loss<float>, dim3(grid), dim3(256), 0, st, (const float*)z, tr, w, b, target, pred, lpx, cls, (unsigned*)hist, P);
+    return loss_select_launch(lpx, cls, state, hist, loss_out, P, grid, true, st);
+}
+
 int ocrs_head_bwd(const void* z, const float* tr, const float* w, const float* pred, const float* gpred, void* gy, double* acc64,
                   const float* saved, double* gsum, long P, int dtype, hipStream_t st) {
     OCRS_CHECK_ARG(gy);
diff --git a/ocrs_models_amd/csrc/loss_optim.hip b/ocrs_models_amd/csrc/loss_optim.hip
--- a/ocrs_models_amd/csrc/loss_optim.hip
+++ b/ocrs_models_amd/csrc/loss_optim.hip
@@ -1,20 +1,6 @@
 #include "common.h"
 
 #include "loss_state.h"
-
-constexpr int LOSS_MAXB = 1024;
-constexpr int LOSS_HIST_WORDS = 2 * 2048;
-struct LossParts {
-    unsigned long long cnt[LOSS_MAXB][2];
-    double sum[LOSS_MAXB][2];
-};
-__device__ __forceinline__ LossParts* loss_parts(unsigned* hist) { return reinterpret_cast<LossParts*>(hist + LOSS_HIST_WORDS); }
-
-__device__ __forceinline__ float log1p_neg(float p) {
-    const float u = 1.f - p;
-    if (u <= 0.f) return -__builtin_inff();
-    return logf(u) - ((u - 1.f) + p) / u;
-}
 
 template <int VEC>
 struct Quad {
@@ -73,10 +59,8 @@
         QuadB<VEC> cq;
 #pragma unroll
         for (int e = 0; e < VEC; ++e) {
-            const float p = pq.v[e], t0 = tq.v[e];
-            const unsigned char c = t0 > 0.5f ? 1 : (t0 < 0.5f ? 2 : 0);
-            const float t = fminf(fmaxf(t0, 0.f), 1.f);
-            lq.v[e] = -(t * fmaxf(logf(p), -100.f) + (1.f - t) * fmaxf(log1p_neg(p), -100.f));
+            const unsigned char c = bce_class(tq.v[e]);
+            lq.v[e] = bce_pixel(pq.v[e], tq.v[e]);
             cq.v[e] = c;
             np += c == 1;
             nn += c == 2;
@@ -89,10 +73,8 @@
     }
     if (VEC > 1 && blockIdx.x == 0 && threadIdx.x < P - nq * VEC) {
         const long i = nq * VEC + threadIdx.x;
-        const float p = pred[i], t0 = target[i];
-        const unsigned char c = t0 > 0.5f ? 1 : (t0 < 0.5f ? 2 : 0);
-        const float t = fminf(fmaxf(t0, 0.f), 1.f);
-        const float l = -(t * fmaxf(logf(p), -100.f) + (1.f - t) * fmaxf(log1p_neg(p), -100.f));
+        const unsigned char c = bce_class(target[i]);
+        const float l = bce_pixel(pred[i], target[i]);
         lpx[i] = l;
         cls[i] = c;
         np += c == 1;
@@ -100,20 +82,7 @@
         if (c) atomicAdd(&s_h[(c - 1) * 2048 + (loss_key(l) >> 20)], 1u);
     }
     __shared__ unsigned s_cnt[2];
-    if (threadIdx.x < 2) s_cnt[threadIdx.x] = 0;
-    __syncthreads();
-    for (int o = 32; o > 0; o >>= 1) {
-        np += __shfl_xor(np, o, 64);
-        nn += __shfl_xor(nn, o, 64);
-    }
-    if ((threadIdx.x & 63) == 0) {
-        atomicAdd(&s_cnt[0], (unsigned)np);
-        atomicAdd(&s_cnt[1], (unsigned)nn);
-    }
-    __syncthreads();
-    if (threadIdx.x < 2) loss_parts(hist)->cnt[blockIdx.x][threadIdx.x] = s_cnt[threadIdx.x];
-    for (int i = threadIdx.x; i < LOSS_HIST_WORDS; i += 256)
-        if (s_h[i]) atomicAdd(&hist[i], s_h[i]);
+    bce_block_finish(np, nn, s_h, s_cnt, hist);
 }
 
 __device__ __forceinline__ void pass_bits(int pass, int& shift, int& nb) {
@@ -185,127 +154,158 @@
     }
 }
 
+__device__ __forceinline__ double tree256_f64(const double* s , int lane) {
+    double x = (s[lane] + s[lane + 128]) + (s[lane + 64] + s[lane + 192]);
+#pragma unroll
+    for (int o = 32; o > 0; o >>= 1) x += __shfl_xor(x, o, 64);
+    return x;
+}
+
 __global__ __launch_bounds__(256) void k_select_scan(LossState* __restrict__ stt, unsigned* __restrict__ hist, int pass, int nblk, float* __restrict__ loss_out) {
-    __shared__ unsigned long long s_sum[256];
-    __shared__ double s_d[256];
-    __shared__ unsigned long long s_need[2], s_ties[2], s_k;
+    __shared__ unsigned long long s_cw[2][4], s_w[2][4];
+    __shared__ double s_d[4][256];
+    __shared__ unsigned long long s_need[2], s_ties[2];
     __shared__ int s_bin[2];
     int shift, nb;
     pass_bits(pass, shift, nb);
     const int per = nb / 256;
-    const int tid = threadIdx.x;
+    const int tid = threadIdx.x, lane = tid & 63, wave = tid >> 6;
     LossParts* lp = loss_parts(hist);
-    auto block_sum_u64 = [&](unsigned long long v) -> unsigned long long {
-        __syncthreads();
-        s_sum[tid] = v;
-        __syncthreads();
-        for (int o = 128; o > 0; o >>= 1) {
-            if (tid < o) s_sum[tid] += s_sum[tid + o];
-            __syncthreads();
-        }
-        return s_sum[0];
-    };
-    auto block_sum_f64 = [&](double v) -> double {
-        __syncthreads();
-        s_d[tid] = v;
-        __syncthreads();
-        for (int o = 128; o > 0; o >>= 1) {
-            if (tid < o) s_d[tid] += s_d[tid + o];
-            __syncthreads();
-        }
-        return s_d[0];
-    };
+    unsigned hv[2][8];
+#pragma unroll
+    for (int c = 0; c < 2; ++c) {
+        const uint4* p = reinterpret_cast<const uint4*>(hist + c * 2048 + nb - (tid + 1) * per);
+        const uint4 a = p[0], b = per == 8 ? p[1] : make_uint4(0, 0, 0, 0);
+        const unsigned up[8] = {a.x, a.y, a.z, a.w, b.x, b.y, b.z, b.w};
+#pragma unroll
+        for (int j = 0; j < 8; ++j) hv[c][j] = per == 8 ? up[7 - j] : (j < 4 ? up[3 - j] : 0u);
+    }
+    unsigned long long need[2] = {0, 0}, k = 0, c0 = 0, c1 = 0;
+    unsigned pfx[2] = {0, 0};
     if (pass == 0) {
-        unsigned long long c0 = 0, c1 = 0;
         for (int b = tid; b < nblk; b += 256) {
-            c0 += lp->cnt[b][0];
-            c1 += lp->cnt[b][1];
-        }
-        const unsigned long long n0 = block_sum_u64(c0), n1 = block_sum_u64(c1);
+            const ulonglong2 v = *reinterpret_cast<const ulonglong2*>(lp->cnt[b]);
+            c0 += v.x;
+            c1 += v.y;
+        }
+    } else {
+        need[0] = stt->need[0];
+        need[1] = stt->need[1];
+        pfx[0] = stt->prefix[0];
+        pfx[1] = stt->prefix[1];
+        k = stt->k;
+    }
+    double2 ab[4];
+#pragma unroll
+    for (int i = 0; i < 4; ++i) {
+        const int b = tid + 256 * i;
+        ab[i] = (pass == 2 && b < nblk) ? *reinterpret_cast<const double2*>(lp->sum[b]) : make_double2(0.0, 0.0);
+    }
+    asm volatile("s_waitcnt vmcnt(0)" ::: "memory");
+    if (pass == 0) {
+#pragma unroll
+        for (int o = 32; o > 0; o >>= 1) {
+            c0 += __shfl_xor(c0, o, 64);
+            c1 += __shfl_xor(c1, o, 64);
+        }
+        if (lane == 0) {
+            s_cw[0][wave] = c0;
+            s_cw[1][wave] = c1;
+        }
+    }
+    unsigned long long loc[2], inc[2];
+#pragma unroll
+    for (int c = 0; c < 2; ++c) {
+        loc[c] = 0;
+#pragma unroll
+        for (int j = 0; j < 8; ++j) loc[c] += hv[c][j];
+        inc[c] = loc[c];
+#pragma unroll
+        for (int o = 1; o < 64; o <<= 1) {
+            const unsigned long long t = __shfl_up(inc[c], o, 64);
+            if (lane >= o) inc[c] += t;
+        }
+        if (lane == 63) s_w[c][wave] = inc[c];
+    }
+    if (tid < 2) s_bin[tid] = -1;
+    __syncthreads();
+    if (pass == 0) {
+        const unsigned long long n0 = (s_cw[0][0] + s_cw[0][1]) + (s_cw[0][2] + s_cw[0][3]), n1 = (s_cw[1][0] + s_cw[1][1]) + (s_cw[1][2] + s_cw[1][3]);
+        k = n0 < n1 ? n0 : n1;
+        need[0] = need[1] = k;
         if (tid == 0) {
-            const unsigned long long k = n0 < n1 ? n0 : n1;
             stt->cnt[0] = n0;
             stt->cnt[1] = n1;
             stt->k = k;
-            s_k = k;
-            for (int c = 0; c < 2; ++c) {
-                stt->prefix[c] = 0;
-                stt->ties[c] = 0;
-                stt->sum_gt[c] = 0.0;
-                s_need[c] = k;
-            }
-        }
-    } else if (tid == 0) {
-        s_need[0] = stt->need[0];
-        s_need[1] = stt->need[1];
-        s_k = stt->k;
-    }
-    if (tid < 2) s_bin[tid] = -1;
-    __syncthreads();
-    double tot = 0.0;
+            stt->sum_gt[0] = stt->sum_gt[1] = 0.0;
+        }
+    }
+#pragma unroll
     for (int c = 0; c < 2; ++c) {
-        unsigned* h = hist + c * 2048;
-        unsigned long long loc = 0;
-        for (int j = 0; j < per; ++j) loc += h[nb - 1 - (tid * per + j)];
-        const unsigned pfx = pass == 0 ? 0u : stt->prefix[c];
-        __syncthreads();
-        s_sum[tid] = loc;
-        __syncthreads();
-        if (tid == 0) {
-            unsigned long long run = 0;
-            for (int t = 0; t < 256; ++t) {
-                const unsigned long long v = s_sum[t];
-                s_sum[t] = run;
-                run += v;
-            }
-        }
-        __syncthreads();
-        const unsigned long long need = s_need[c];
-        const unsigned long long before = s_sum[tid];
-        if (need > 0 && before < need && before + loc >= need) {
+        unsigned long long before = inc[c] - loc[c];
+        for (int w = 0; w < wave; ++w) before += s_w[c][w];
+        if (need[c] > 0 && before < need[c] && before + loc[c] >= need[c]) {
             unsigned long long run = before;
-            for (int j = 0; j < per; ++j) {
-                const int bin = nb - 1 - (tid * per + j);
-                const unsigned long long v = h[bin];
-                if (run + v >= need) {
-                    stt->prefix[c] = (pfx << (pass == 0 ? 11 : 10)) | (unsigned)bin;
-                    stt->need[c] = need - run;
+            bool found = false;
+#pragma unroll
+            for (int j = 0; j < 8; ++j) {
+                const unsigned long long v = hv[c][j];
+                if (!found && j < per && run + v >= need[c]) {
+                    const int bin = nb - 1 - (tid * per + j);
+                    stt->prefix[c] = (pfx[c] << (pass == 0 ? 11 : 10)) | (unsigned)bin;
+                    stt->need[c] = need[c] - run;
                     stt->ties[c] = v;
-                    s_need[c] = need - run;
+                    s_need[c] = need[c] - run;
                     s_ties[c] = v;
                     s_bin[c] = bin;
-                    break;
+                    found = true;
                 }
                 run += v;
             }
-        } else if (need == 0 && tid == 0) {
+        } else if (need[c] == 0 && tid == 0) {
             stt->need[c] = 0;
-        }
-        __syncthreads();
-        if (pass == 2) {
-            const int bin = s_bin[c];
-            const unsigned long long ties = bin >= 0 ? s_ties[c] : 0ull, needc = bin >= 0 ? s_need[c] : 0ull;
-            const unsigned thr = bin >= 0 ? ((pfx << 10) | (unsigned)bin) : pfx;
-            double in_b = 0.0;
-            if (bin >= 0)
-                for (int j = 0; j < per; ++j) {
-                    const int bj = nb - 1 - (tid * per + j);
-                    if (bj > bin && h[bj]) in_b += (double)h[bj] * (double)__uint_as_float((pfx << 10) | (unsigned)bj);
-                }
-            double above = 0.0;
-            for (int b = tid; b < nblk; b += 256) above += lp->sum[b][c];
-            const double sum_gt = block_sum_f64(above) + block_sum_f64(in_b);
-            if (tid == 0) {
-                stt->sum_gt[c] = sum_gt;
-                stt->frac[c] = ties ? (float)((double)needc / (double)ties) : 0.f;
+            if (pass == 0) {
+                stt->prefix[c] = 0;
+                stt->ties[c] = 0;
             }
-            tot += sum_gt + (double)needc * (double)__uint_as_float(thr);
-        }
-        __syncthreads();
+        }
     }
     for (int i = tid; i < LOSS_HIST_WORDS; i += 256) hist[i] = 0;
-    if (pass == 2 && tid == 0) {
-        const unsigned long long k = s_k;
+    if (pass != 2) return;
+    __syncthreads();
+    int bin[2];
+#pragma unroll
+    for (int c = 0; c < 2; ++c) {
+        bin[c] = s_bin[c];
+        double in_b = 0.0;
+        if (bin[c] >= 0)
+#pragma unroll
+            for (int j = 0; j < 8; ++j) {
+                const int bj = nb - 1 - (tid * per + j);
+                if (j < per && bj > bin[c] && hv[c][j]) in_b += (double)hv[c][j] * (double)__uint_as_float((pfx[c] << 10) | (unsigned)bj);
+            }
+        double above = 0.0;
+#pragma unroll
+        for (int i = 0; i < 4; ++i)
+            if (tid + 256 * i < nblk) above += c == 0 ? ab[i].x : ab[i].y;
+        s_d[2 * c][tid] = above;
+        s_d[2 * c + 1][tid] = in_b;
+    }
+    __syncthreads();
+    if (wave != 0) return;
+    double tot = 0.0;
+#pragma unroll
+    for (int c = 0; c < 2; ++c) {
+        const unsigned long long ties = bin[c] >= 0 ? s_ties[c] : 0ull, needc = bin[c] >= 0 ? s_need[c] : 0ull;
+        const unsigned thr = bin[c] >= 0 ? ((pfx[c] << 10) | (unsigned)bin[c]) : pfx[c];
+        const double sum_gt = tree256_f64(s_d[2 * c], lane) + tree256_f64(s_d[2 * c + 1], lane);
+        if (tid == 0) {
+            stt->sum_gt[c] = sum_gt;
+            stt->frac[c] = ties ? (float)((double)needc / (double)ties) : 0.f;
+        }
+        tot += sum_gt + (double)needc * (double)__uint_as_float(thr);
+    }
+    if (tid == 0) {
         const float loss = k ? (float)(tot / (2.0 * (double)k)) : __uint_as_float(0x7fc00000u);
         stt->loss = loss;
         stt->inv2k = k ? (float)(1.0 / (2.0 * (double)k)) : 0.f;
@@ -429,6 +429,21 @@
     for (int i = threadIdx.x; i < n; i += 64) dst[d + i] = (float)((double)dst[d + i] + src[s0 + i]);
 }
 
+int loss_select_launch(const float* lpx, const unsigned char* cls, void* state, void* hist, float* loss_out, long P, int grid, bool vec, hipStream_t st) {
+    LossState* stt = (LossState*)state;
+    for (int pass = 0; pass < 3; ++pass) {
+        if (pass > 0) {
+            if (vec)
+                hipLaunchKernelGGL(k_select_hist<4>, dim3(grid), dim3(256), 0, st, lpx, cls, stt, (unsigned*)hist, pass, P);
+            else
+                hipLaunchKernelGGL(k_select_hist<1>, dim3(grid), dim3(256), 0, st, lpx, cls, stt, (unsigned*)hist, pass, P);
+        }
+        hipLaunchKernelGGL(k_select_scan, dim3(1), dim3(256), 0, st, stt, (unsigned*)hist, pass, grid, loss_out);
+    }
+    OCRS_LAUNCH_CHECK();
+    return OCRS_OK;
+}
+
 extern "C" {
 
 long ocrs_loss_state_bytes() { return (long)sizeof(LossState); }
@@ -436,8 +451,7 @@
 
 int ocrs_balanced_bce_fwd(const float* pred, const float* target, float* lpx, unsigned char* cls, void* state, void* hist, float* loss_out,
                           long P, hipStream_t st) {
-    OCRS_CHECK_ARG(pred && target && lpx && cls && state && hist && loss_out && P > 0);
-    LossState* stt = (LossState*)state;
+    OCRS_CHECK_ARG(pred && target && lpx && cls && state && hist && aligned16(hist) && loss_out && P > 0);
     if (hipMemsetAsync(hist, 0, LOSS_HIST_WORDS * sizeof(unsigned), st) != hipSuccess) return OCRS_ERR_HIP;
     int grid = ew_grid((P + 3) / 4);
     if (grid > LOSS_MAXB) grid = LOSS_MAXB;
@@ -447,15 +461,12 @@
         hipLaunchKernelGGL(k_bce_fwd<4>, dim3(grid), dim3(256), 0, st, pred, target, lpx, cls, (unsigned*)hist, P);
     else
         hipLaunchKernelGGL(k_bce_fwd<1>, dim3(grid), dim3(256), 0, st, pred, target, lpx, cls, (unsigned*)hist, P);
-    for (int pass = 0; pass < 3; ++pass) {
-        if (pass > 0) {
-            if (vec)
-                hipLaunchKernelGGL(k_select_hist<4>, dim3(grid), dim3(256), 0, st, lpx, cls, stt, (unsigned*)hist, pass, P);
-            else
-                hipLaunchKernelGGL(k_select_hist<1>, dim3(grid), dim3(256), 0, st, lpx, cls, stt, (unsigned*)hist, pass, P);
-        }
-        hipLaunchKernelGGL(k_select_scan, dim3(1), dim3(256), 0, st, stt, (unsigned*)hist, pass, grid, loss_out);
-    }
+    return loss_select_launch(lpx, cls, state, hist, loss_out, P, grid, vec, st);
+}
+
+int ocrs_select_scan(void* state, void* hist, int pass, int nblk, float* loss_out, hipStream_t st) {
+    OCRS_CHECK_ARG(state && hist && aligned16(hist) && loss_out && pass >= 0 && pass <= 2 && nblk > 0 && nblk <= LOSS_MAXB);
+    hipLaunchKernelGGL(k_select_scan, dim3(1), dim3(256), 0, st, (LossState*)state, (unsigned*)hist, pass, nblk, loss_out);
     OCRS_LAUNCH_CHECK();
     return OCRS_OK;
 }
diff --git a/ocrs_models_amd/csrc/loss_state.h b/ocrs_models_amd/csrc/loss_state.h
--- a/ocrs_models_amd/csrc/loss_state.h
+++ b/ocrs_models_amd/csrc/loss_state.h
@@ -12,3 +12,43 @@
 };
 
 __device__ __forceinline__ unsigned loss_key(float v) { return __float_as_uint(v) & 0x7fffffffu; }
+
+constexpr int LOSS_MAXB = 1024;
+constexpr int LOSS_HIST_WORDS = 2 * 2048;
+struct LossParts {
+    unsigned long long cnt[LOSS_MAXB][2];
+    double sum[LOSS_MAXB][2];
+};
+__device__ __forceinline__ LossParts* loss_parts(unsigned* hist) { return reinterpret_cast<LossParts*>(hist + LOSS_HIST_WORDS); }
+
+__device__ __forceinline__ float log1p_neg(float p) {
+    const float u = 1.f - p;
+    if (u <= 0.f) return -__builtin_inff();
+    return logf(u) - ((u - 1.f) + p) / u;
+}
+
+__device__ __forceinline__ unsigned char bce_class(float t0) { return t0 > 0.5f ? 1 : (t0 < 0.5f ? 2 : 0); }
+__device__ __forceinline__ float bce_pixel(float p, float t0) {
+    const float t = fminf(fmaxf(t0, 0.f), 1.f);
+    return -(t * fmaxf(logf(p), -100.f) + (1.f - t) * fmaxf(log1p_neg(p), -100.f));
+}
+
+__device__ __forceinline__ void bce_block_finish(unsigned long long np, unsigned long long nn, const unsigned* s_h, unsigned* s_cnt,
+                                                 unsigned* __restrict__ hist) {
+    if (threadIdx.x < 2) s_cnt[threadIdx.x] = 0;
+    __syncthreads();
+    for (int o = 32; o > 0; o >>= 1) {
+        np += __shfl_xor(np, o, 64);
+        nn += __shfl_xor(nn, o, 64);
+    }
+    if ((threadIdx.x & 63) == 0) {
+        atomicAdd(&s_cnt[0], (unsigned)np);
+        atomicAdd(&s_cnt[1], (unsigned)nn);
+    }
+    __syncthreads();
+    if (threadIdx.x < 2) loss_parts(hist)->cnt[blockIdx.x][threadIdx.x] = s_cnt[threadIdx.x];
+    for (int i = threadIdx.x; i < LOSS_HIST_WORDS; i += 256)
+        if (s_h[i]) atomicAdd(&hist[i], s_h[i]);
+}
+
+int loss_select_launch(const float* lpx, const unsigned char* cls, void* state, void* hist, float* loss_out, long P, int grid, bool vec, hipStream_t st);
diff --git a/ocrs_models_amd/ddp.py b/ocrs_models_amd/ddp.py
--- a/ocrs_models_amd/ddp.py
+++ b/ocrs_models_amd/ddp.py
@@ -82,12 +82,26 @@
                     dist.broadcast(t, src=0, group=process_group)
         module._grad_bucketer = self.bucketer
 
-    def forward(self, *args, **kwargs):
+    def _sync_buffers(self):
         if self.broadcast_buffers and dist.is_initialized() and dist.get_world_size(self.pg) > 1:
             with torch.no_grad():
                 for b in self.module.buffers():
                     dist.broadcast(b, src=0, group=self.pg)
+
+    def forward(self, *args, **kwargs):
+        self._sync_buffers()
         return self.module(*args, **kwargs)
+
+    @property
+    def forward_loss(self):
+        inner = getattr(self.module, "forward_loss", None)
+        if inner is None:
+            return None
+
+        def forward_loss(*args, **kwargs):
+            self._sync_buffers()
+            return inner(*args, **kwargs)
+        return forward_loss
 
     def state_dict(self, *a, **k):
         return self.module.state_dict(*a, **k)
diff --git a/ocrs_models_amd/losses.py b/ocrs_models_amd/losses.py
--- a/ocrs_models_amd/losses.py
+++ b/ocrs_models_amd/losses.py
@@ -55,21 +55,25 @@
     return gpred
 
 
+def loss_buffers(P: int, dev):
+    L = lib()
+    return (torch.empty(P, dtype=torch.float32, device=dev), torch.empty(P, dtype=torch.uint8, device=dev),
+            torch.empty(L.loss_state_bytes(), dtype=torch.uint8, device=dev), torch.empty(L.loss_hist_bytes(), dtype=torch.uint8, device=dev),
+            torch.empty((), dtype=torch.float32, device=dev))
+
+
 class _BalancedBCE(torch.autograd.Function):
     @staticmethod
-    def forward(ctx, pred, target):
-        L = lib()
+    def forward(ctx, pred, target, pre=None):
         ctx.from_det = type(pred.grad_fn).__name__ == "_DetFnBackward" and pred.is_contiguous() and pred.dtype == torch.float32
         pred = pred.contiguous().float()
-        target = target.contiguous().float()
-        P = pred.numel()
-        dev = pred.device
-        lpx = torch.empty(P, dtype=torch.float32, device=dev)
-        cls = torch.empty(P, dtype=torch.uint8, device=dev)
-        state = torch.empty(L.loss_state_bytes(), dtype=torch.uint8, device=dev)
-        hist = torch.empty(L.loss_hist_bytes(), dtype=torch.uint8, device=dev)
-        loss = torch.empty((), dtype=torch.float32, device=dev)
-        L.balanced_bce_fwd(ptr(pred), ptr(target), ptr(lpx), ptr(cls), ptr(state), ptr(hist), ptr(loss), P)
+        if pre is not None:
+            target, lpx, cls, state, loss = pre
+        else:
+            target = target.contiguous().float()
+            P = pred.numel()
+            lpx, cls, state, hist, loss = loss_buffers(P, pred.device)
+            lib().balanced_bce_fwd(ptr(pred), ptr(target), ptr(lpx), ptr(cls), ptr(state), ptr(hist), ptr(loss), P)
         ctx.save_for_backward(pred, target, lpx, cls, state)
         return loss
 
@@ -80,10 +84,10 @@
         key = (pred.device.index, pred.data_ptr())
         if _FUSE["on"] and ctx.from_det and key not in _PENDING:
             _PENDING[key] = (pred, target, lpx, cls, state, g)
-            return _zero_marker(pred.device).expand(pred.shape), None
+            return _zero_marker(pred.device).expand(pred.shape), None, None
         gpred = torch.empty_like(pred)
         lib().balanced_bce_bwd(ptr(pred), ptr(target), ptr(lpx), ptr(cls), ptr(state), ptr(g), ptr(gpred), pred.numel())
-        return gpred, None
+        return gpred, None, None
 
 
 def balanced_cross_entropy_loss(pred: torch.Tensor, target: torch.Tensor) -> torch.Tensor:
diff --git a/ocrs_models_amd/models.py b/ocrs_models_amd/models.py
--- a/ocrs_models_amd/models.py
+++ b/ocrs_models_amd/models.py
@@ -87,12 +87,13 @@
 
     overlap = True
     use_mm = use_rs32 = fuse_bn_bwd = fold_fwd_fin = True
-    c1_u = c1_noz = c1_fuse = head_gl = True
+    c1_u = c1_noz = c1_fuse = head_gl = head_loss = True
     packs = EMPTY_PACKS
     _zpool, _zoff = None, 0
     _flat, _folds, _defer_folds = None, (), False
     _keep_ws, _deferring = None, False
     _head_gl = _c1acc = None
+    loss_target = loss_pre = None
 
     def __init__(self, P, Bf, dev, dtype, N, train=True, mod=None, x=None):
         self.L = lib()
@@ -332,7 +333,15 @@
             up = self.double(f"up.{i}.contract", ta, skip, Cout)
         pred = self.empty(N, 1, H, W, dtype=torch.float32)
         up.other_use = True
-        L.head_fwd(ptr(up.t), ptr(up.tr), ptr(P["out_conv.0.weight"]), ptr(P["out_conv.0.bias"]), ptr(pred), N * H * W, self.dt)
+        head = (ptr(up.t), ptr(up.tr), ptr(P["out_conv.0.weight"]), ptr(P["out_conv.0.bias"]))
+        tgt, self.loss_target = self.loss_target, None
+        if tgt is not None and self.head_loss and (N * H * W) % 4 == 0 and all(t.data_ptr() % 16 == 0 for t in (up.t, tgt, pred)):
+            from . import losses as _losses
+            lpx, cls, state, hist, loss = _losses.loss_buffers(N * H * W, self.dev)
+            L.head_fwd_loss(*head, ptr(tgt), ptr(pred), ptr(lpx), ptr(cls), ptr(state), ptr(hist), ptr(loss), N * H * W, self.dt)
+            self.loss_pre = (tgt, lpx, cls, state, loss)
+        else:
+            L.head_fwd(*head, ptr(pred), N * H * W, self.dt)
         self.head_in, self.pred, self.skips, self.HW = up, pred, skips, (H, W)
         return pred
 
@@ -661,6 +670,20 @@
         return torch.float32
 
     def forward(self, x: torch.Tensor) -> torch.Tensor:
+        return self._forward(x, None)[0]
+
+    def forward_loss(self, x: torch.Tensor, target: torch.Tensor):
+        from . import losses as _losses
+
+        if x.dim() == 4 and x.shape[1] == 1 and target.shape != x.shape:
+            raise RuntimeError(f"pred {tuple(x.shape)} and target {tuple(target.shape)} must have the same shape")
+        tgt = target.contiguous().float() if target.is_cuda else None
+        pred, pre = self._forward(x, tgt)
+        if pre is None:
+            return pred, _losses.balanced_cross_entropy_loss(pred, target)
+        return pred, _losses._BalancedBCE.apply(pred, target, pre)
+
+    def _forward(self, x, loss_target):
         if not x.is_cuda:
             raise RuntimeError("ocrs_models_amd.DetectionModel runs on MI355X only (no CPU path); move the model and input to 'cuda'")
         if x.dim() != 4 or x.shape[1] != 1:
@@ -673,6 +696,10 @@
                 raise RuntimeError("parameters must be contiguous fp32")
         run = _DetRun(dict(zip(names, (p.detach() for p in params))), dict(self.named_buffers()), x.device, self._act_dtype(), x.shape[0],
                       self.training, mod=self, x=x)
+        run.loss_target = loss_target
         if torch.is_grad_enabled() and any(p.requires_grad for p in params):
-            return _DetFn.apply(run, *params)
-        return run.forward()
+            pred = _DetFn.apply(run, *params)
+        else:
+            pred = run.forward()
+        pre, run.loss_pre = run.loss_pre, None
+        return pred, pre
diff --git a/ocrs_models_amd/train_detection.py b/ocrs_models_amd/train_detection.py
--- a/ocrs_models_amd/train_detection.py
+++ b/ocrs_models_amd/train_detection.py
@@ -19,8 +19,12 @@
 def train_step(model, optimizer, batch: dict, device, loss_fn=balanced_cross_entropy_loss) -> torch.Tensor:
     img = batch["image"].to(device, non_blocking=True)
     masks = batch["text_mask"].to(device, non_blocking=True)
-    pred_masks = model(img)
-    loss = loss_fn(pred_masks, masks)
+    forward_loss = getattr(model, "forward_loss", None) if loss_fn is balanced_cross_entropy_loss else None
+    if forward_loss is not None:
+        pred_masks, loss = forward_loss(img, masks)
+    else:
+        pred_masks = model(img)
+        loss = loss_fn(pred_masks, masks)
     optimizer.zero_grad()
     if loss_fn is balanced_cross_entropy_loss:
         with fused_head_backward():
```
